# FuxiComputerVision/Nefii

Hardware: AMD Instinct MI355X
Metric: training rays/sec (Step-2 material opt) (higher is better)
Workload: dtype f16x3; 1 GPU; cfg3; parallelism=dp1, trace_tier=True, bracket_staged_eval=False, split_fp8=False, step_graph=False, cycle_batches=4, trace_prefetch=3, nonfinite_steps=0

## Files before the change

### include/nefii_amd.h

```cpp
#ifndef NEFII_AMD_H
#define NEFII_AMD_H

#include <stddef.h>
#include <stdint.h>

#ifdef __cplusplus
extern "C" {
#endif

#define NEFII_ABI_VERSION 18
#define NEFII_MAX_LAYERS 12
#define NEFII_TILE_ROWS 32
#define NEFII_MAX_WIDTH 512
#define NEFII_MAX_ENC 96
#define NEFII_MAX_LOBES 512

enum { NEFII_ACT_RELU = 0, NEFII_ACT_ELU = 1, NEFII_ACT_SOFTPLUS100 = 2 };
enum { NEFII_HEAD_NONE = 0, NEFII_HEAD_TANH01 = 1, NEFII_HEAD_POW2 = 2, NEFII_HEAD_SIGMOID = 3,
       NEFII_HEAD_RELU = 4, NEFII_HEAD_ABS = 5, NEFII_HEAD_RELU_INIT = 6 };
enum { NEFII_E_ARG = -1, NEFII_E_SHAPE = -2, NEFII_E_UNSUPPORTED = -3 };

typedef struct nefii_layer {
    int32_t k_x, k_e;
    int32_t n_out;
    int32_t n_pad;
    const float *w_fwd;
    const float *w_bwd;
    const float *bias;
    const void *w_f16x3;
    const void *w_bwd_f16x3;
} nefii_layer;

typedef struct nefii_mlp {
    int32_t n_layers;
    int32_t act;
    int32_t head;
    int32_t enc_freqs[3];
    int32_t feat_width;
    int32_t reserved;
    const void *w_stream;
    nefii_layer layer[NEFII_MAX_LAYERS];
} nefii_mlp;

int nefii_abi_version(void);

int nefii_padded_width(int v);

int nefii_pack_linear(const float *W, const float *bias, int n_out, int k_in,
                      int x_src0, int x_len, int e_src0, int e_len, float scale,
                      float *w_fwd, float *w_bwd, float *bias_pad, void *stream);

int nefii_pack_linear_f16x3(const float *W, int n_out, int k_in, int x_src0, int x_len, int e_src0, int e_len,
                            float scale, void *w_f16x3, void *stream);

typedef struct nefii_pack_source {
    const float *W;
    const float *bias;
    int32_t n_out, k_in, x_src0, x_len, e_src0, e_len;
    float scale;
    int32_t skip_f32;
} nefii_pack_source;
int nefii_pack_mlp(const nefii_mlp *h_mlp, const nefii_pack_source *h_layers, void *stream);

int nefii_mlp_forward(const nefii_mlp *h_mlp, const float *in_a, const float *in_b, const float *in_c,
                      const float *feat, int64_t n, float *out, int out_stride,
                      float *hidden_out, int hid_stride, float *stash, int stash_stride, void *stream);

int nefii_mlp_backward(const nefii_mlp *h_mlp, const float *d_out, int out_stride, const float *stash,
                       int stash_stride, int64_t n, float *dz, int dz_stride, void *stream);

int nefii_mlp_wgrad(const float *dz, int dz_stride, const float *x, int x_stride, int64_t n, int n_out, int k_in,
                    float scale, float *dW, float *db, void *stream);

int nefii_mlp_forward_f16(const nefii_mlp *h_mlp, const float *in_a, const float *in_b, const float *in_c,
                          const float *feat, int64_t n, float *out, int out_stride,
                          float *hidden_out, int hid_stride, float *stash, int stash_stride, int single_pass,
                          void *stream);
int nefii_mlp_grad_scale(const float *d_out, int64_t count, float *scale, void *stream);
int nefii_mlp_grad_scale_head(const float *d_out, int out_stride, const float *pre, int pre_stride, int64_t n, int n_out,
                              int head, float *scale, void *stream);
int nefii_mlp_backward_f16(const nefii_mlp *h_mlp, const float *d_out, int out_stride, const float *stash,
                           int stash_stride, int64_t n, float *dz, int dz_stride, const float *scale, void *stream);
int nefii_mlp_wgrad_f16(const float *dz, int dz_stride, const float *x, int x_stride, int64_t n, int n_out, int k_in,
                        float scale, const float *gscale, float *dW, float *db, void *stream);

int nefii_mlp_h16_supported(const nefii_mlp *h_mlp);
int nefii_mlp_x0_width(const nefii_mlp *h_mlp);
int nefii_mlp_forward_f16h(const nefii_mlp *h_mlp, const float *in_a, const float *in_b, const float *in_c,
                           const float *feat, int64_t n, float *out, int out_stride, float *hidden_out, int hid_stride,
                           void *stash16, int stash_stride, float *z_last, void *x0_16, void *stream);
int nefii_mlp_backward_f16h(const nefii_mlp *h_mlp, const float *d_out, int out_stride, const void *stash16,
                            int stash_stride, const float *z_last, int64_t n, void *dz16, int dz_stride,
                            const float *scale, void *stream);
int nefii_mlp_wgrad_f16h(const void *dz16, int dz_stride, const void *x, int x_stride, int x_half, int64_t n, int n_out,
                         int k_in, float scale, const float *gscale, float *dW, float *db, void *stream);

#define NEFII_MAX_WGRAD_ITEMS 12
typedef struct nefii_wgrad_item {
    const void *dz16;
    const void *x;
    float *dW, *db;
    int32_t dz_stride, x_stride, x_half, n_out, k_in;
    float scale;
} nefii_wgrad_item;
int nefii_mlp_wgrad_f16h_batch(const nefii_wgrad_item *h_items, int n_items, int64_t n, const float *gscale, void *stream);

int nefii_encode_inputs(const nefii_mlp *h_mlp, const float *in_a, const float *in_b, const float *in_c,
                        const float *feat, int64_t n, float *out, int width, void *stream);

int nefii_sdf_value_grad(const nefii_mlp *h_mlp, const float *x, int64_t n, float *sdf_out, int out_stride,
                         float *feat_out, int feat_stride, float *grad_out, float *ws, void *stream);
size_t nefii_sdf_value_grad_workspace_bytes(const nefii_mlp *h_mlp, int64_t n);

typedef struct nefii_tracer_params {
    float object_bounding_sphere, sdf_threshold, line_search_step;
    int32_t line_step_iters, sphere_tracing_iters, n_steps, n_rootfind_steps;
    int32_t training;
    int32_t bisect_levels;
    int32_t precision;
    float coarse_tau;
    int32_t coarse_cap;
    int32_t minsdf_group;
    int32_t small_round;
    int32_t trace_tier;
    float tier_kappa;
    float tier_gate;
    float minsdf_lipschitz;
    int32_t unread_misses;
    int32_t split_fp8;
} nefii_tracer_params;
#define NEFII_TRACE_COUNTERS 14
#define NEFII_CNT_SINGLES 0
#define NEFII_CNT_DENSE_ROWS 1
#define NEFII_CNT_BISECT_RAYS 2
#define NEFII_CNT_BISECT_USED 3
#define NEFII_CNT_REFINED 4
#define NEFII_CNT_COARSE_WINDOWS 5
#define NEFII_CNT_SEARCHES 6
#define NEFII_CNT_BISECT_EVALS 7
#define NEFII_CNT_TAU_AUDIT 8
#define NEFII_CNT_COARSE_SINGLES 9
#define NEFII_CNT_REPEATS 10
#define NEFII_CNT_COARSE_SAMPLES 11
#define NEFII_CNT_LIP_AUDIT 12
#define NEFII_CNT_PROBES 13

size_t nefii_sdf_stream_bytes(const nefii_mlp *h_sdf);
int nefii_pack_sdf_stream(const nefii_mlp *h_sdf, void *w_stream, void *stream);

size_t nefii_mlp_stream_bytes(const nefii_mlp *h_mlp);
int nefii_pack_mlp_stream(const nefii_mlp *h_mlp, void *w_stream, void *stream);

int nefii_pack_linear_f16x3_bwd(const float *W, int n_out, int k_in, int x_src0, int x_len, int e_src0, int e_len,
                                float scale, void *w_bwd_f16x3, void *stream);

int nefii_sdf_eval(const nefii_mlp *h_sdf, const float *x, int64_t n, float *sdf_out, void *stream);
int nefii_sdf_eval_coarse(const nefii_mlp *h_sdf, const float *x, int64_t n, float *sdf_out, void *stream);
int nefii_sdf_coarse_supported(const nefii_mlp *h_sdf);
int nefii_sdf_eval_fp8corr(const nefii_mlp *h_sdf, const float *x, int64_t n, float *sdf_out, void *stream);
int nefii_sdf_fp8corr_supported(const nefii_mlp *h_sdf);

size_t nefii_trace_workspace_bytes(int64_t n_rays, const nefii_tracer_params *h_params);
int nefii_trace_max_rounds(const nefii_tracer_params *h_params);
int nefii_trace_rays(const nefii_mlp *h_sdf, const nefii_tracer_params *h_params,
                     const float *origins, const float *dirs, const uint8_t *object_mask, int64_t n_rays,
                     const float *lin_steps, const float *minsdf_steps,
                     float *out_points, uint8_t *out_hit, float *out_dists,
                     void *workspace, size_t workspace_bytes, int32_t *counters, void *stream);

int nefii_trace_rays_rounds(const nefii_mlp *h_sdf, const nefii_tracer_params *h_params,
                            const float *origins, const float *dirs, const uint8_t *object_mask, int64_t n_rays,
                            const float *lin_steps, const float *minsdf_steps,
                            float *out_points, uint8_t *out_hit, float *out_dists,
                            void *workspace, size_t workspace_bytes, int32_t *counters,
                            int round_begin, int round_end, void *stream);
int nefii_trace_rays_groups(const nefii_mlp *h_sdf, const nefii_tracer_params *h_params,
                            const float *origins, const float *dirs, const uint8_t *object_mask,
                            int n_groups, const int64_t *group_begin,
                            const float *lin_steps, const float *minsdf_steps,
                            float *out_points, uint8_t *out_hit, float *out_dists,
                            void *const *workspaces, const size_t *workspace_bytes, int32_t *counters,
                            int round_begin, int round_end, void *const *streams);

#define NEFII_BOUND_GRID_MAX 640
size_t nefii_sdf_bound_grid_workspace_bytes(int G);
int nefii_sdf_bound_grid_build(const nefii_mlp *h_sdf, int G, float radius, float tau, float L_floor, float safety,
                               void *out_cells, void *workspace, void *stream);
int nefii_trace_rays_rounds_grid(const nefii_mlp *h_sdf, const nefii_tracer_params *h_params,
                                 const float *origins, const float *dirs, const uint8_t *object_mask, int64_t n_rays,
                                 const float *lin_steps, const float *minsdf_steps,
                                 float *out_points, uint8_t *out_hit, float *out_dists,
                                 void *workspace, size_t workspace_bytes, int32_t *counters,
                                 int round_begin, int round_end, const void *cells, int G, void *stream);
int nefii_trace_rays_groups_grid(const nefii_mlp *h_sdf, const nefii_tracer_params *h_params,
                                 const float *origins, const float *dirs, const uint8_t *object_mask,
                                 int n_groups, const int64_t *group_begin,
                                 const float *lin_steps, const float *minsdf_steps,
                                 float *out_points, uint8_t *out_hit, float *out_dists,
                                 void *const *workspaces, const size_t *workspace_bytes, int32_t *counters,
                                 int round_begin, int round_end, const void *cells, int G, void *const *streams);

int nefii_trace_profile_enable(int on);
int nefii_trace_profile_read(double *h_eval_ms, int *h_n_eval, double *h_span_ms);
int nefii_trace_profile_launches(float *h_ms, int cap);

int nefii_camera_rays(const float *uv, const float *pose, const float *intrinsics, int batch, int64_t samples,
                      float *out_dirs, float *out_origins, void *stream);


int nefii_sg_render_forward(const float *lgtSGs, int n_lobes, const float *specular, const float *roughness,
                            const float *albedo, const float *normal, const float *view, int64_t n,
                            float *rgb, float *spec_rgb, float *diff_rgb, void *stream);
int nefii_sg_render_backward(const float *lgtSGs, int n_lobes, const float *specular, const float *roughness,
                             const float *albedo, const float *normal, const float *view, int64_t n,
                             const float *d_rgb, const float *d_spec, const float *d_diff,
                             float *g_albedo, float *g_roughness, float *g_specular, float *g_lgtSGs, void *stream);

int nefii_env_radiance_forward(const float *lgtSGs, int n_lobes, const float *dirs, int64_t n, float eps,
                               float *rgb, void *stream);
int nefii_env_radiance_backward(const float *lgtSGs, int n_lobes, const float *dirs, int64_t n, float eps,
                                const float *d_rgb, float *g_lgtSGs, void *stream);

int64_t nefii_envfit_workspace_bytes(int64_t n, int n_lobes);
int nefii_envfit_loss_grad(const float *lgtSGs, int n_lobes, const float *dirs, const float *target, int64_t n, float eps,
                           void *workspace, float *loss, float *g_lgtSGs, float *rgb, void *stream);
int nefii_envfit_adam(float *lgtSGs, float *exp_avg, float *exp_avg_sq, int n_lobes, const float *dirs,
                      const float *target, int64_t n, float eps, double lr, double beta1, double beta2,
                      double adam_eps, int64_t step0, int iters, void *workspace, float *losses, void *stream);

int64_t nefii_mcubes_workspace_bytes(int nx, int ny, int nz);
int nefii_mcubes_count(const float *vol, int nx, int ny, int nz, float level, void *workspace, int64_t *counts,
                       void *stream);
int nefii_mcubes_emit(const float *vol, int nx, int ny, int nz, float level, float origin_x, float origin_y,
                      float origin_z, float spacing_x, float spacing_y, float spacing_z, void *workspace, float *verts,
                      int64_t max_verts, int *faces, int64_t max_tris, void *stream);

int nefii_mis_sample(const float *lgtSGs, int n_lobes, const float *roughness, const float *normal, const float *view,
                     const float *uniforms, int64_t n, float *wi, float *own_pdf, float *pdf_table, void *stream);

int64_t nefii_envlight_table_bytes(int height, int width);
int nefii_envlight_build(const float *map, int height, int width, void *table, void *stream);
int nefii_envlight_mis_sample(const float *map, const void *table, int height, int width, int coord,
                              const float *roughness, const float *normal, const float *view, const float *uniforms,
                              int64_t n, float *wi, float *own_pdf, float *pdf_table, float *light, void *stream);
int nefii_envlight_radiance(const float *map, int height, int width, int coord, const float *dirs, int64_t n,
                            float *rgb, void *stream);
int nefii_envlight_pdf(const void *table, int height, int width, int coord, const float *dirs, int64_t n, float *pdf,
                       void *stream);

int nefii_envlight_bounce_sample(const float *map, const void *table, int height, int width, int coord,
                                 const float *specular, const float *roughness, const float *albedo,
                                 const float *normal, const float *view, const float *uniforms, int64_t m, float *wo,
                                 float *weight, float *mix_pdf, void *stream);

int nefii_envlight_mis_sample_rot(const float *map, const void *table, int height, int width, int coord,
                                  const float *rot, const int *rot_identity, int A, const float *roughness,
                                  const float *normal, const float *view, const float *uniforms, int64_t n, float *wi,
                                  float *own_pdf, float *pdf_table, float *light, void *stream);
int nefii_envlight_bounce_sample_rot(const float *map, const void *table, int height, int width, int coord,
                                     const float *rot, const int *rot_identity, int A, const int *rot_index,
                                     const float *specular, const float *roughness, const float *albedo,
                                     const float *normal, const float *view, const float *uniforms, int64_t m,
                                     float *wo, float *weight, float *mix_pdf, void *stream);
int nefii_envlight_radiance_rot(const float *map, int height, int width, int coord, const float *rot,
                                const int *rot_identity, int A, const int *rot_index, const float *dirs, int64_t n,
                                float *rgb, void *stream);
int nefii_envlight_pdf_rot(const void *table, int height, int width, int coord, const float *rot,
                           const int *rot_identity, int A, const int *rot_index, const float *dirs, int64_t n,
                           float *pdf, void *stream);

int nefii_denoise_atrous(const void *guides0, const void *guides1, const void *in, void *out, int n_signals, int height,
                         int width, int step, float sigma_n, float sigma_x, float sigma_c_level, void *stream);

int nefii_mesh_sdf_query(const double *node_box, int64_t n_leaves_pow2, const double *tris ,
                         int64_t n_tris, int leaf_size, const double *points, int64_t n_points, int want_sign, double *out,
                         void *stream);

int nefii_mesh_cc_init(int32_t *parent, int64_t n_verts, int32_t *flags, void *stream);
int nefii_mesh_cc_round(const int32_t *faces, int64_t n_faces, int32_t *parent, int64_t n_verts, int32_t *flags,
                        void *stream);

int nefii_mesh_cluster_quadrics(const float *verts, int64_t n_verts, const int32_t *faces, int64_t n_faces,
                                const int32_t *cluster, const int32_t *corners, const int64_t *seg, const double *centre,
                                int64_t n_clusters, double h, double eps, double clamp, float *pos, int32_t *flags,
                                void *stream);

int64_t nefii_image_metrics_workspace_bytes(int B, int H, int W, int C, int levels);
int nefii_image_metrics(const float *x, const float *y, int B, int H, int W, int C, int levels, const double *window,
                        double c1, double c2, void *workspace, double *stats, double *sq_err, void *stream);

int nefii_mc_shade_forward(const float *specular, const float *roughness, const float *albedo, const float *normal,
                           const float *view, const float *wi, const float *own_pdf, const float *pdf_table,
                           const float *light, const float *visibility, const float *indirect, int64_t n,
                           float *rgb, float *spec_rgb, float *diff_rgb, void *stream);
int nefii_mc_shade_backward(const float *specular, const float *roughness, const float *albedo, const float *normal,
                            const float *view, const float *wi, const float *own_pdf, const float *pdf_table,
                            const float *light, const float *visibility, const float *indirect, int64_t n,
                            const float *d_rgb, const float *d_spec, const float *d_diff, float *g_light,
                            float *g_indirect, float *g_albedo, float *g_roughness, float *g_specular, void *stream);

typedef struct nefii_loss_params {
    float idr_rgb_weight, sg_rgb_weight, mask_weight, alpha, normalsmooth_weight, background_rgb_weight;
    int32_t loss_type;
    int32_t env_loss_type;
    int32_t r_patch;
    int32_t reserved;
} nefii_loss_params;
int nefii_idr_loss(const nefii_loss_params *h_params, const float *idr_rgb, const float *sg_rgb, const float *rgb_gt,
                   const uint8_t *network_object_mask, const uint8_t *object_mask, const float *sdf_output,
                   const float *normals, int64_t n, float *losses, float *d_idr_rgb, float *d_sg_rgb, void *stream);

#define NEFII_PATCH_WINDOW 11
typedef struct nefii_patch_loss_params {
    float idr_ssim_weight, sg_ssim_weight, roughnesssmooth_weight;
    int32_t r_patch;
    float window[NEFII_PATCH_WINDOW];
    int32_t reserved;
} nefii_patch_loss_params;
int64_t nefii_idr_patch_loss_workspace_bytes(const nefii_patch_loss_params *h_params, int64_t n);
int nefii_idr_patch_loss(const nefii_patch_loss_params *h_params, const float *idr_rgb, const float *sg_rgb,
                         const float *rgb_gt, const uint8_t *network_object_mask, const uint8_t *object_mask,
                         const float *roughness, const float *normals, int64_t n, void *workspace, float *losses,
                         float *d_idr_rgb, float *d_sg_rgb, float *d_roughness, void *stream);

#define NEFII_MAX_ROW_BLOCKS 12
typedef struct nefii_row_block {
    const float *src;
    float *dst;
    int32_t cols;
    int32_t src_row_stride;
    float fill;
    int32_t reserved;
} nefii_row_block;
int nefii_assemble_rows(const nefii_row_block *h_blocks, int n_blocks, const int64_t *where, int64_t n_src, int64_t rows,
                        void *stream);
int nefii_gather_rows(const nefii_row_block *h_blocks, int n_blocks, const int64_t *where, int64_t n_src, int64_t rows,
                      void *stream);

int nefii_prepare_hits(const float *points, const float *ray_dirs, const float *grad, const float *feat_src, int feat_cols,
                       const int64_t *where, int64_t n, int64_t rows, float *pts_out, float *view_out, float *nrm_out,
                       float *feat_out, void *stream);

int nefii_material_head_global(const float *rough_param, const float *spec_param, int n_spec, int fake_rough, int fake_spec,
                               float *rough_out, float *spec_out, void *stream);
int nefii_material_head_global_backward(const float *rough_param, const float *spec_param, int n_spec, int fake_rough,
                                        int fake_spec, const float *d_rough, const float *d_spec, float *g_rough_param,
                                        float *g_spec_param, void *stream);

int nefii_mfma_sustained_probe(int groups, float *h_ms, double *h_flops, void *stream);
int nefii_mfma_sustained_probe_chains(int groups, int chains, float *h_ms, double *h_flops, void *stream);

#ifdef __cplusplus
}
#endif
#endif
```

### nefii_amd/_lib.py

```python
import ctypes
import os

HERE = os.path.dirname(os.path.abspath(__file__))
LIB_PATH = os.environ.get('NEFII_LIB_PATH', os.path.join(HERE, 'csrc', 'libnefii_hip.so'))

MAX_LAYERS = 12
TILE_ROWS = 32
MAX_WIDTH = 512
MAX_ENC = 96
ABI_VERSION = 18
TRACE_COUNTERS = 14
(CNT_SINGLES, CNT_DENSE_ROWS, CNT_BISECT_RAYS, CNT_BISECT_USED, CNT_REFINED, CNT_COARSE_WINDOWS, CNT_SEARCHES, CNT_BISECT_EVALS,
 CNT_TAU_AUDIT, CNT_COARSE_SINGLES, CNT_REPEATS, CNT_COARSE_SAMPLES, CNT_LIP_AUDIT, CNT_PROBES) = range(TRACE_COUNTERS)
CNT_WORK = [CNT_SINGLES, CNT_DENSE_ROWS, CNT_BISECT_RAYS, CNT_REFINED, CNT_COARSE_WINDOWS, CNT_COARSE_SINGLES, CNT_COARSE_SAMPLES]
CNT_MAXIMA = [CNT_TAU_AUDIT, CNT_LIP_AUDIT]
TRACE_WS_FLOAT_ARRAYS = 13
TRACE_ITER_SHIFT = 20

ACT_RELU, ACT_ELU, ACT_SOFTPLUS100 = 0, 1, 2
HEAD_NONE, HEAD_TANH01, HEAD_POW2, HEAD_SIGMOID, HEAD_RELU, HEAD_ABS, HEAD_RELU_INIT = range(7)

c_float_p = ctypes.c_void_p


class Layer(ctypes.Structure):
    _fields_ = [('k_x', ctypes.c_int32), ('k_e', ctypes.c_int32), ('n_out', ctypes.c_int32),
                ('n_pad', ctypes.c_int32), ('w_fwd', ctypes.c_void_p), ('w_bwd', ctypes.c_void_p),
                ('bias', ctypes.c_void_p), ('w_f16x3', ctypes.c_void_p), ('w_bwd_f16x3', ctypes.c_void_p)]


class Mlp(ctypes.Structure):
    _fields_ = [('n_layers', ctypes.c_int32), ('act', ctypes.c_int32), ('head', ctypes.c_int32),
                ('enc_freqs', ctypes.c_int32 * 3), ('feat_width', ctypes.c_int32), ('reserved', ctypes.c_int32),
                ('w_stream', ctypes.c_void_p), ('layer', Layer * MAX_LAYERS)]


class TracerParams(ctypes.Structure):
    _fields_ = [('object_bounding_sphere', ctypes.c_float), ('sdf_threshold', ctypes.c_float),
                ('line_search_step', ctypes.c_float), ('line_step_iters', ctypes.c_int32),
                ('sphere_tracing_iters', ctypes.c_int32), ('n_steps', ctypes.c_int32),
                ('n_rootfind_steps', ctypes.c_int32), ('training', ctypes.c_int32), ('bisect_levels', ctypes.c_int32),
                ('precision', ctypes.c_int32), ('coarse_tau', ctypes.c_float), ('coarse_cap', ctypes.c_int32),
                ('minsdf_group', ctypes.c_int32), ('small_round', ctypes.c_int32), ('trace_tier', ctypes.c_int32),
                ('tier_kappa', ctypes.c_float), ('tier_gate', ctypes.c_float), ('minsdf_lipschitz', ctypes.c_float),
                ('unread_misses', ctypes.c_int32), ('split_fp8', ctypes.c_int32)]


class PackSource(ctypes.Structure):
    _fields_ = [('W', ctypes.c_void_p), ('bias', ctypes.c_void_p), ('n_out', ctypes.c_int32), ('k_in', ctypes.c_int32),
                ('x_src0', ctypes.c_int32), ('x_len', ctypes.c_int32), ('e_src0', ctypes.c_int32), ('e_len', ctypes.c_int32),
                ('scale', ctypes.c_float), ('skip_f32', ctypes.c_int32)]


class WgradItem(ctypes.Structure):
    _fields_ = [('dz16', ctypes.c_void_p), ('x', ctypes.c_void_p), ('dW', ctypes.c_void_p), ('db', ctypes.c_void_p),
                ('dz_stride', ctypes.c_int32), ('x_stride', ctypes.c_int32), ('x_half', ctypes.c_int32),
                ('n_out', ctypes.c_int32), ('k_in', ctypes.c_int32), ('scale', ctypes.c_float)]


MAX_WGRAD_ITEMS = 12


class RowBlock(ctypes.Structure):
    _fields_ = [('src', ctypes.c_void_p), ('dst', ctypes.c_void_p), ('cols', ctypes.c_int32), ('src_row_stride', ctypes.c_int32),
                ('fill', ctypes.c_float), ('reserved', ctypes.c_int32)]


MAX_ROW_BLOCKS = 12


class LossParams(ctypes.Structure):
    _fields_ = [('idr_rgb_weight', ctypes.c_float), ('sg_rgb_weight', ctypes.c_float), ('mask_weight', ctypes.c_float),
                ('alpha', ctypes.c_float), ('normalsmooth_weight', ctypes.c_float),
                ('background_rgb_weight', ctypes.c_float), ('loss_type', ctypes.c_int32),
                ('env_loss_type', ctypes.c_int32), ('r_patch', ctypes.c_int32), ('reserved', ctypes.c_int32)]


PATCH_WINDOW = 11


class PatchLossParams(ctypes.Structure):
    _fields_ = [('idr_ssim_weight', ctypes.c_float), ('sg_ssim_weight', ctypes.c_float),
                ('roughnesssmooth_weight', ctypes.c_float), ('r_patch', ctypes.c_int32),
                ('window', ctypes.c_float * PATCH_WINDOW), ('reserved', ctypes.c_int32)]


P = ctypes.c_void_p
I = ctypes.c_int
I64 = ctypes.c_int64
F = ctypes.c_float
D = ctypes.c_double

SIGNATURES = {
    'nefii_abi_version': (I, []),
    'nefii_padded_width': (I, [I]),
    'nefii_pack_linear': (I, [P, P, I, I, I, I, I, I, F, P, P, P, P]),
    'nefii_pack_linear_f16x3': (I, [P, I, I, I, I, I, I, F, P, P]),
    'nefii_pack_linear_f16x3_bwd': (I, [P, I, I, I, I, I, I, F, P, P]),
    'nefii_pack_mlp': (I, [ctypes.POINTER(Mlp), ctypes.POINTER(PackSource), P]),
    'nefii_mlp_forward': (I, [ctypes.POINTER(Mlp), P, P, P, P, I64, P, I, P, I, P, I, P]),
    'nefii_mlp_backward': (I, [ctypes.POINTER(Mlp), P, I, P, I, I64, P, I, P]),
    'nefii_mlp_wgrad': (I, [P, I, P, I, I64, I, I, F, P, P, P]),
    'nefii_mlp_forward_f16': (I, [ctypes.POINTER(Mlp), P, P, P, P, I64, P, I, P, I, P, I, I, P]),
    'nefii_mlp_grad_scale': (I, [P, I64, P, P]),
    'nefii_mlp_grad_scale_head': (I, [P, I, P, I, I64, I, I, P, P]),
    'nefii_mlp_backward_f16': (I, [ctypes.POINTER(Mlp), P, I, P, I, I64, P, I, P, P]),
    'nefii_mlp_wgrad_f16': (I, [P, I, P, I, I64, I, I, F, P, P, P, P]),
    'nefii_mlp_h16_supported': (I, [ctypes.POINTER(Mlp)]),
    'nefii_mlp_x0_width': (I, [ctypes.POINTER(Mlp)]),
    'nefii_mlp_forward_f16h': (I, [ctypes.POINTER(Mlp), P, P, P, P, I64, P, I, P, I, P, I, P, P, P]),
    'nefii_mlp_backward_f16h': (I, [ctypes.POINTER(Mlp), P, I, P, I, P, I64, P, I, P, P]),
    'nefii_mlp_wgrad_f16h': (I, [P, I, P, I, I, I64, I, I, F, P, P, P, P]),
    'nefii_mlp_wgrad_f16h_batch': (I, [ctypes.POINTER(WgradItem), I, I64, P, P]),
    'nefii_encode_inputs': (I, [ctypes.POINTER(Mlp), P, P, P, P, I64, P, I, P]),
    'nefii_sdf_value_grad': (I, [ctypes.POINTER(Mlp), P, I64, P, I, P, I, P, P, P]),
    'nefii_sdf_value_grad_workspace_bytes': (ctypes.c_size_t, [ctypes.POINTER(Mlp), I64]),
    'nefii_sdf_stream_bytes': (ctypes.c_size_t, [ctypes.POINTER(Mlp)]),
    'nefii_pack_sdf_stream': (I, [ctypes.POINTER(Mlp), P, P]),
    'nefii_mlp_stream_bytes': (ctypes.c_size_t, [ctypes.POINTER(Mlp)]),
    'nefii_pack_mlp_stream': (I, [ctypes.POINTER(Mlp), P, P]),
    'nefii_sdf_eval': (I, [ctypes.POINTER(Mlp), P, I64, P, P]),
    'nefii_sdf_eval_coarse': (I, [ctypes.POINTER(Mlp), P, I64, P, P]),
    'nefii_sdf_coarse_supported': (I, [ctypes.POINTER(Mlp)]),
    'nefii_sdf_eval_fp8corr': (I, [ctypes.POINTER(Mlp), P, I64, P, P]),
    'nefii_sdf_fp8corr_supported': (I, [ctypes.POINTER(Mlp)]),
    'nefii_trace_workspace_bytes': (ctypes.c_size_t, [I64, ctypes.POINTER(TracerParams)]),
    'nefii_trace_max_rounds': (I, [ctypes.POINTER(TracerParams)]),
    'nefii_trace_rays': (I, [ctypes.POINTER(Mlp), ctypes.POINTER(TracerParams), P, P, P, I64, P, P, P, P, P, P,
                             ctypes.c_size_t, P, P]),
    'nefii_trace_rays_rounds': (I, [ctypes.POINTER(Mlp), ctypes.POINTER(TracerParams), P, P, P, I64, P, P, P, P, P, P,
                                    ctypes.c_size_t, P, I, I, P]),
    'nefii_trace_rays_groups': (I, [ctypes.POINTER(Mlp), ctypes.POINTER(TracerParams), P, P, P, I, P, P, P, P, P, P, P, P,
                                    P, I, I, P]),
    'nefii_sdf_bound_grid_workspace_bytes': (ctypes.c_size_t, [I]),
    'nefii_sdf_bound_grid_build': (I, [ctypes.POINTER(Mlp), I, F, F, F, F, P, P, P]),
    'nefii_trace_rays_rounds_grid': (I, [ctypes.POINTER(Mlp), ctypes.POINTER(TracerParams), P, P, P, I64, P, P, P, P, P, P,
                                         ctypes.c_size_t, P, I, I, P, I, P]),
    'nefii_trace_rays_groups_grid': (I, [ctypes.POINTER(Mlp), ctypes.POINTER(TracerParams), P, P, P, I, P, P, P, P, P, P, P, P,
                                         P, I, I, P, I, P]),
    'nefii_trace_profile_enable': (I, [I]),
    'nefii_trace_profile_read': (I, [ctypes.POINTER(ctypes.c_double), ctypes.POINTER(I), ctypes.POINTER(ctypes.c_double)]),
    'nefii_trace_profile_launches': (I, [ctypes.POINTER(ctypes.c_float), I]),
    'nefii_idr_loss': (I, [ctypes.POINTER(LossParams), P, P, P, P, P, P, P, I64, P, P, P, P]),
    'nefii_idr_patch_loss_workspace_bytes': (I64, [ctypes.POINTER(PatchLossParams), I64]),
    'nefii_idr_patch_loss': (I, [ctypes.POINTER(PatchLossParams), P, P, P, P, P, P, P, I64, P, P, P, P, P, P]),
    'nefii_camera_rays': (I, [P, P, P, I, I64, P, P, P]),
    'nefii_assemble_rows': (I, [ctypes.POINTER(RowBlock), I, P, I64, I64, P]),
    'nefii_gather_rows': (I, [ctypes.POINTER(RowBlock), I, P, I64, I64, P]),
    'nefii_prepare_hits': (I, [P, P, P, P, I, P, I64, I64, P, P, P, P, P]),
    'nefii_material_head_global': (I, [P, P, I, I, I, P, P, P]),
    'nefii_material_head_global_backward': (I, [P, P, I, I, I, P, P, P, P, P]),
    'nefii_sg_render_forward': (I, [P, I, P, P, P, P, P, I64, P, P, P, P]),
    'nefii_sg_render_backward': (I, [P, I, P, P, P, P, P, I64, P, P, P, P, P, P, P, P]),
    'nefii_env_radiance_forward': (I, [P, I, P, I64, F, P, P]),
    'nefii_env_radiance_backward': (I, [P, I, P, I64, F, P, P, P]),
    'nefii_envfit_workspace_bytes': (I64, [I64, I]),
    'nefii_envfit_loss_grad': (I, [P, I, P, P, I64, F, P, P, P, P, P]),
    'nefii_envfit_adam': (I, [P, P, P, I, P, P, I64, F, D, D, D, D, I64, I, P, P, P]),
    'nefii_mcubes_workspace_bytes': (I64, [I, I, I]),
    'nefii_mcubes_count': (I, [P, I, I, I, F, P, P, P]),
    'nefii_mcubes_emit': (I, [P, I, I, I, F, F, F, F, F, F, F, P, P, I64, P, I64, P]),
    'nefii_mis_sample': (I, [P, I, P, P, P, P, I64, P, P, P, P]),
    'nefii_envlight_table_bytes': (I64, [I, I]),
    'nefii_envlight_build': (I, [P, I, I, P, P]),
    'nefii_envlight_mis_sample': (I, [P, P, I, I, I, P, P, P, P, I64, P, P, P, P, P]),
    'nefii_envlight_bounce_sample': (I, [P, P, I, I, I, P, P, P, P, P, P, I64, P, P, P, P]),
    'nefii_envlight_radiance': (I, [P, I, I, I, P, I64, P, P]),
    'nefii_envlight_pdf': (I, [P, I, I, I, P, I64, P, P]),
    'nefii_envlight_mis_sample_rot': (I, [P, P, I, I, I, P, P, I, P, P, P, P, I64, P, P, P, P, P]),
    'nefii_envlight_bounce_sample_rot': (I, [P, P, I, I, I, P, P, I, P, P, P, P, P, P, P, I64, P, P, P, P]),
    'nefii_envlight_radiance_rot': (I, [P, I, I, I, P, P, I, P, P, I64, P, P]),
    'nefii_envlight_pdf_rot': (I, [P, I, I, I, P, P, I, P, P, I64, P, P]),
    'nefii_denoise_atrous': (I, [P, P, P, P, I, I, I, I, F, F, F, P]),
    'nefii_image_metrics_workspace_bytes': (I64, [I, I, I, I, I]),
    'nefii_image_metrics': (I, [P, P, I, I, I, I, I, ctypes.POINTER(D), D, D, P, P, P, P]),
    'nefii_mesh_sdf_query': (I, [P, I64, P, I64, I, P, I64, I, P, P]),
    'nefii_mesh_cc_init': (I, [P, I64, P, P]),
    'nefii_mesh_cc_round': (I, [P, I64, P, I64, P, P]),
    'nefii_mesh_cluster_quadrics': (I, [P, I64, P, I64, P, P, P, P, I64, D, D, D, P, P, P]),
    'nefii_mc_shade_forward': (I, [P] * 11 + [I64, P, P, P, P]),
    'nefii_mc_shade_backward': (I, [P] * 11 + [I64] + [P] * 9),
    'nefii_mfma_sustained_probe': (I, [I, ctypes.POINTER(ctypes.c_float), ctypes.POINTER(ctypes.c_double), P]),
    'nefii_mfma_sustained_probe_chains': (I, [I, I, ctypes.POINTER(ctypes.c_float), ctypes.POINTER(ctypes.c_double), P]),
}

_lib = None


class NefiiLibraryError(RuntimeError):
    pass


def lib():
    global _lib
    if _lib is not None:
        return _lib
    if not os.path.exists(LIB_PATH):
        raise NefiiLibraryError(
            'libnefii_hip.so is not built (%s missing). Run `python -m nefii_amd.build`. '
            'There is no CPU/PyTorch fallback for the hot path.' % LIB_PATH)
    import torch
    try:
        handle = ctypes.CDLL(LIB_PATH)
    except OSError as e:
        raise NefiiLibraryError('cannot load %s: %s' % (LIB_PATH, e))
    for name, (res, args) in SIGNATURES.items():
        try:
            fn = getattr(handle, name)
        except AttributeError:
            raise NefiiLibraryError('%s does not export %s' % (LIB_PATH, name))
        fn.restype = res
        fn.argtypes = args
    if handle.nefii_abi_version() != ABI_VERSION:
        raise NefiiLibraryError('ABI version mismatch')
    _lib = handle
    return _lib


def check(rc, what):
    if rc != 0:
        raise RuntimeError('%s failed with status %d (%s)' % (
            what, rc, {-1: 'bad argument', -2: 'bad shape', -3: 'unsupported'}.get(rc, 'hipError_t')))
```

### nefii_amd/csrc/nefii_tracer.hip

```cpp
#include <cstdlib>
#include <vector>

#include "mlp_tile.h"
#include "hip_check.h"

using namespace nefii;

namespace {

enum Phase : int { PH_DONE = 0, PH_TRACE = 1, PH_SAMPLER = 2, PH_BISECT = 3, PH_MINSDF = 4, PH_SAMPLER_C = 5, PH_MINSDF_C = 6,
                   PH_SAMPLER_X = 7 };
constexpr int PH_POST = 100, PH_WAIT = -1;
constexpr int NCNT = NEFII_TRACE_COUNTERS;
constexpr int NEAR_PROBES = 6;
enum Kind : int { Q_START = 0, Q_END = 1, Q_MID = 2 };

constexpr int TRACE_WS_FLOAT_ARRAYS = 13, TRACE_ITER_SHIFT = 20;
struct RayState {
    float *t_s, *t_e, *cur_s, *cur_e, *nxt_s, *nxt_e, *t_min, *t_max, *res_s, *res_e, *lo, *hi, *mid;
    int *flags;
    float *big;
    unsigned *singles;
    unsigned *dense;
    unsigned *tri;
    unsigned *cdense;
    unsigned *refine;
    unsigned *csingles;
    int *block_live;
    unsigned *crefine;
    unsigned char *ord;
};
constexpr int CREF_CAP = 76;

constexpr int F_PHASE = 0x7;
constexpr int F_LIVE_S = 1 << 3, F_LIVE_E = 1 << 4, F_PEND_S = 1 << 5, F_PEND_E = 1 << 6;
constexpr int F_STEPPED = 1 << 7;
constexpr int F_SPH = 1 << 8, F_SAMP = 1 << 9, F_HIT = 1 << 10;
constexpr int F_OWN = 1 << 11;
constexpr int F_IT_SHIFT = 12, F_IT_MASK = 0xFF;
constexpr int F_K_SHIFT = TRACE_ITER_SHIFT, F_K_MASK = 0xF;
constexpr int F_WIN_SHIFT = 24, F_WIN_MASK = 0x7;
enum SamplerWin : int {
    SW_WHOLE_ROW = 0,
    SW_WINDOW_1 = 1, SW_WINDOW_2 = 2, SW_WINDOW_3 = 3, SW_WINDOW_4 = 4,
    SW_STAGE1 = 5, SW_STAGE2 = 6,
    SW_GRID = 7
};
enum MinSdfWin : int {
    MW_ROW_IN = 0,
    MW_SECOND = 1,
    MW_STAGE1 = 2, MW_STAGE2 = 3,
    MW_ENTER = 4,
    MW_SHARED = 5
};
__device__ __forceinline__ int win_of(int fl) { return (fl >> F_WIN_SHIFT) & F_WIN_MASK; }
__device__ __forceinline__ int with_win(int fl, int w) { return (fl & ~(F_WIN_MASK << F_WIN_SHIFT)) | (w << F_WIN_SHIFT); }
constexpr int CWIN_STAGE1 = 4;
constexpr int F_CRS_S = 1 << 27, F_CRS_E = 1 << 28, F_AUD_S = 1 << 29, F_AUD_E = 1 << 30;
__host__ __device__ __forceinline__ int coarse_window(int n_steps) { return (n_steps + 3) >> 2; }

__device__ __forceinline__ float fmul(float a, float b) { return __fmul_rn(a, b); }
__device__ __forceinline__ float fadd(float a, float b) { return __fadd_rn(a, b); }
__device__ __forceinline__ float fsub(float a, float b) { return __fsub_rn(a, b); }

struct Params {
    nefii_tracer_params p;
    int64_t n;
    const float *o, *d;
    const uint8_t *obj;
    const float *lin, *steps;
    float *out_pts, *out_dist;
    uint8_t *out_hit;
    int *counters;
    int levels, tri_nodes;
    float tau;
    int cap;
    int chunk;
    float chunk_gate;
    int window;
    float tier_band;
    float tier_gate;
    float lip;
    int share;
    int stage_bracket;
    int miss_argmin;
    const unsigned *cells;
    int grid_n;
    float grid_inv_h;
    RayState s;
};

__host__ __device__ __forceinline__ int stage1_count(int ns) { return coarse_window(ns); }
__host__ __device__ __forceinline__ int stage1_pos(int ns, int j) { return (j * (ns - 1)) / (stage1_count(ns) - 1); }
__device__ __forceinline__ bool staged_bracket(const Params &P, int64_t r) {
    return P.lip > 0.f && P.stage_bracket && (!P.p.training || P.obj[r] == 0);
}
__device__ __forceinline__ int minsdf_row(const Params &P, int64_t r) {
    const int g = P.p.minsdf_group;
    return g > 0 ? (int)(r / g) : 0;
}

__device__ __forceinline__ float minsdf_step(const Params &P, int64_t r, int i) {
    const int g = P.p.minsdf_group;
    return P.steps[(g > 0 ? (r / g) * (int64_t)P.p.n_steps : 0) + i];
}

struct Emit {
    bool qs, qe;
    bool cs, ce;
    bool qt, qd;
    int nc, cwin;
    unsigned dense_which;
    int consumed;
    int n_alg;
    int n_ref;
    unsigned cmask[4];
    int n_rep;
    bool ref_coarse;
    __device__ __forceinline__ void mark(int i) {
#pragma unroll
        for (int w = 0; w < 4; ++w) cmask[w] |= (i >> 5) == w ? 1u << (i & 31) : 0u;
    }
    __device__ __forceinline__ bool marked(int i) const {
        unsigned word = 0u;
#pragma unroll
        for (int w = 0; w < 4; ++w) word = (i >> 5) == w ? cmask[w] : word;
        return (word >> (i & 31)) & 1u;
    }
    __device__ __forceinline__ void clear_marks() { cmask[0] = cmask[1] = cmask[2] = cmask[3] = 0u; }
};
enum Total : int { T_SINGLES, T_DENSE, T_TRI, T_CONSUMED, T_REFINE, T_CWINDOWS, T_ALG, T_CSINGLES, T_REP, T_CREFINE, N_TOTALS };
enum List : int { L_SINGLES, L_DENSE, L_TRI, L_REFINE, L_CDENSE, L_CSINGLES, L_CREFINE, N_LISTS };

__device__ __forceinline__ void append_queries(const Params &P, int round, unsigned ray, const Emit &e) {
    __shared__ int wtot[N_TOTALS][4];
    __shared__ int base[N_LISTS];
    const bool qs = e.qs && !e.cs, qe = e.qe && !e.ce, qcs = e.qs && e.cs, qce = e.qe && e.ce;
    const int nc = e.nc, n_ref = e.n_ref;
    const bool ref_coarse = e.ref_coarse;
    const int lane = threadIdx.x & 63, wave = threadIdx.x >> 6;
    const unsigned long long bs = __ballot(qs), be = __ballot(qe), bt = __ballot(e.qt), bd = __ballot(e.qd);
    const unsigned long long bcs = __ballot(qcs), bce = __ballot(qce);
    const unsigned long long lt = (1ull << lane) - 1ull;
    int cons = e.consumed, alg = e.n_alg, rep = e.n_rep;
#pragma unroll
    for (int o = 32; o > 0; o >>= 1) cons += __shfl_xor(cons, o), alg += __shfl_xor(alg, o), rep += __shfl_xor(rep, o);
    int incl = ref_coarse ? 0 : n_ref;
    int incl2 = ref_coarse ? n_ref : 0;
#pragma unroll
    for (int o = 1; o < 64; o <<= 1) {
        const int t = __shfl_up(incl, o), t2 = __shfl_up(incl2, o);
        if (lane >= o) incl += t, incl2 += t2;
    }
    const int wref = __shfl(incl, 63), wref2 = __shfl(incl2, 63);
    int cincl = nc;
#pragma unroll
    for (int o = 1; o < 64; o <<= 1) {
        const int t = __shfl_up(cincl, o);
        if (lane >= o) cincl += t;
    }
    const int wcoarse = __shfl(cincl, 63);
    if (lane == 0) {
        wtot[T_SINGLES][wave] = __popcll(bs) + __popcll(be);
        wtot[T_DENSE][wave] = __popcll(bd);
        wtot[T_TRI][wave] = __popcll(bt);
        wtot[T_CONSUMED][wave] = cons;
        wtot[T_REFINE][wave] = wref;
        wtot[T_CWINDOWS][wave] = wcoarse;
        wtot[T_ALG][wave] = alg;
        wtot[T_CSINGLES][wave] = __popcll(bcs) + __popcll(bce);
        wtot[T_REP][wave] = rep;
        wtot[T_CREFINE][wave] = wref2;
    }
    __syncthreads();
    if (threadIdx.x == 0) {
        int t[N_TOTALS];
        for (int i = 0; i < N_TOTALS; ++i) t[i] = wtot[i][0] + wtot[i][1] + wtot[i][2] + wtot[i][3];
        int *cnt = P.counters + round * NCNT;
        base[L_SINGLES] = t[T_SINGLES] ? atomicAdd(&cnt[NEFII_CNT_SINGLES], t[T_SINGLES]) : 0;
        base[L_DENSE] = t[T_DENSE] ? atomicAdd(&cnt[NEFII_CNT_DENSE_ROWS], t[T_DENSE]) : 0;
        base[L_TRI] = t[T_TRI] ? atomicAdd(&cnt[NEFII_CNT_BISECT_RAYS], t[T_TRI]) : 0;
        if (t[T_CONSUMED]) atomicAdd(&cnt[NEFII_CNT_BISECT_USED], t[T_CONSUMED]);
        base[L_REFINE] = t[T_REFINE] ? atomicAdd(&cnt[NEFII_CNT_REFINED], t[T_REFINE]) : 0;
        base[L_CDENSE] = t[T_CWINDOWS] ? atomicAdd(&cnt[NEFII_CNT_COARSE_WINDOWS], t[T_CWINDOWS]) : 0;
        if (t[T_ALG]) atomicAdd(&cnt[NEFII_CNT_SEARCHES], t[T_ALG]);
        if (t[T_TRI]) atomicAdd(&cnt[NEFII_CNT_BISECT_EVALS], t[T_TRI] * P.tri_nodes);
        base[L_CSINGLES] = t[T_CSINGLES] ? atomicAdd(&cnt[NEFII_CNT_COARSE_SINGLES], t[T_CSINGLES]) : 0;
        if (t[T_REP]) atomicAdd(&cnt[NEFII_CNT_REPEATS], t[T_REP]);
        base[L_CREFINE] = t[T_CREFINE] ? atomicAdd(&cnt[NEFII_CNT_COARSE_SAMPLES], t[T_CREFINE]) : 0;
    }
    __syncthreads();
    int off_s = base[L_SINGLES], off_d = base[L_DENSE], off_t = base[L_TRI], off_r = base[L_REFINE], off_c = base[L_CDENSE],
        off_cs = base[L_CSINGLES], off_r2 = base[L_CREFINE];
    for (int w = 0; w < wave; ++w) {
        off_r2 += wtot[T_CREFINE][w];
        off_s += wtot[T_SINGLES][w];
        off_d += wtot[T_DENSE][w];
        off_t += wtot[T_TRI][w];
        off_r += wtot[T_REFINE][w];
        off_c += wtot[T_CWINDOWS][w];
        off_cs += wtot[T_CSINGLES][w];
    }
    if (qs) P.s.singles[off_s + __popcll(bs & lt)] = (ray << 2) | Q_START;
    if (qe) P.s.singles[off_s + __popcll(bs) + __popcll(be & lt)] = (ray << 2) | Q_END;
    if (qcs) P.s.csingles[off_cs + __popcll(bcs & lt)] = (ray << 2) | Q_START;
    if (qce) P.s.csingles[off_cs + __popcll(bcs) + __popcll(bce & lt)] = (ray << 2) | Q_END;
    if (e.qd) P.s.dense[off_d + __popcll(bd & lt)] = (ray << 1) | e.dense_which;
    if (e.qt) P.s.tri[off_t + __popcll(bt & lt)] = ray;
    for (int k = 0; k < nc; ++k)
        P.s.cdense[off_c + cincl - nc + k] = ((unsigned)(e.cwin + k) << 29) | (ray << 1) | e.dense_which;
    if (n_ref > 0) {
        size_t o = ref_coarse ? (size_t)off_r2 + incl2 - n_ref : (size_t)off_r + incl - n_ref;
        unsigned *list = ref_coarse ? P.s.crefine : P.s.refine;
#pragma unroll
        for (int w = 0; w < 4; ++w) {
            unsigned mbits = e.cmask[w];
            while (mbits) {
                const int bit = __ffs(mbits) - 1;
                mbits &= mbits - 1;
                list[o++] = (ray << 7) | (unsigned)(32 * w + bit);
            }
        }
    }
    __syncthreads();
}

__device__ __forceinline__ float tri_depth(float lo, float hi, int j) {
    const unsigned k = (unsigned)j + 1u;
    const int level = 31 - __clz(k);
    float mid = fmul(fadd(lo, hi), 0.5f);
    for (int b = level - 1; b >= 0; --b) {
        if ((k >> b) & 1u) lo = mid; else hi = mid;
        mid = fmul(fadd(lo, hi), 0.5f);
    }
    return mid;
}

__device__ __forceinline__ void finish(const Params &P, int64_t r, float dist, bool hit) {
    const float ox = P.o[r * 3], oy = P.o[r * 3 + 1], oz = P.o[r * 3 + 2];
    const float dx = P.d[r * 3], dy = P.d[r * 3 + 1], dz = P.d[r * 3 + 2];
    P.out_dist[r] = dist;
    P.out_hit[r] = hit ? 1 : 0;
    P.out_pts[r * 3] = fadd(ox, fmul(dist, dx));
    P.out_pts[r * 3 + 1] = fadd(oy, fmul(dist, dy));
    P.out_pts[r * 3 + 2] = fadd(oz, fmul(dist, dz));
}

__global__ __launch_bounds__(128) void minsdf_order_kernel(Params P) {
    const int ns = P.p.n_steps, i = threadIdx.x;
    if (i >= ns) return;
    const float *st = P.steps + (size_t)blockIdx.x * ns;
    const float si = st[i];
    int rank = 0;
    for (int j = 0; j < ns; ++j) {
        const float sj = st[j];
        rank += (sj < si || (sj == si && j < i)) ? 1 : 0;
    }
    P.s.ord[(size_t)blockIdx.x * ns + rank] = (unsigned char)i;
}


__device__ __forceinline__ int init_ray(const Params &P, int64_t r, int round, int &fl, Emit &e) {
    const bool tier = P.tier_band > 0.f;
    const float ox = P.o[r * 3], oy = P.o[r * 3 + 1], oz = P.o[r * 3 + 2];
    const float dx = P.d[r * 3], dy = P.d[r * 3 + 1], dz = P.d[r * 3 + 2];
    const float b = fadd(fadd(fmul(dx, ox), fmul(dy, oy)), fmul(dz, oz));
    const float nrm = sqrtf(fadd(fadd(fmul(ox, ox), fmul(oy, oy)), fmul(oz, oz)));
    const float rad = P.p.object_bounding_sphere;
    const float under = fsub(fmul(b, b), fsub(fmul(nrm, nrm), fmul(rad, rad)));
    const bool sph = under > 0.f;
    float t0 = 0.f, t1 = 0.f;
    if (sph) {
        const float sq = sqrtf(under);
        t0 = fmaxf(fsub(-sq, b), 0.01f);
        t1 = fmaxf(fsub(sq, b), 0.01f);
    }
    P.s.t_s[r] = t0;
    P.s.t_e[r] = t1;
    P.s.t_min[r] = t0;
    P.s.t_max[r] = t1;
    P.s.nxt_s[r] = 0.f;
    P.s.nxt_e[r] = 0.f;
    P.s.cur_s[r] = 0.f;
    P.s.cur_e[r] = 0.f;
    fl = PH_TRACE;
    if (!sph) return PH_TRACE;
    fl |= F_SPH | F_LIVE_S | F_LIVE_E | F_PEND_S | F_PEND_E;
    e.qs = e.qe = true;
    e.cs = tier && t0 > 0.01f;
    e.ce = tier && t1 > 0.01f;
    fl |= (e.cs ? F_CRS_S : 0) | (e.ce ? F_CRS_E : 0);
    P.s.flags[r] = fl;
    return PH_WAIT;
}

__device__ __forceinline__ void begin_stage1(const Params &P, int64_t r, int from, int stage_code, int &fl, Emit &e) {
    float *v = P.s.big + (size_t)r * P.p.n_steps;
    for (int i = from; i < P.p.n_steps; ++i) v[i] = __builtin_inff();
    e.nc = 1;
    e.cwin = CWIN_STAGE1;
    fl = with_win(fl, stage_code);
}

__device__ __forceinline__ bool grid_bounds(const Params &P, int64_t r, float t, float &lo, float &hi) {
    const float rad = P.p.object_bounding_sphere, g = (float)P.grid_n;
    const float ox = P.o[r * 3], oy = P.o[r * 3 + 1], oz = P.o[r * 3 + 2];
    const float dx = P.d[r * 3], dy = P.d[r * 3 + 1], dz = P.d[r * 3 + 2];
    const float fx = fmul(fadd(fadd(ox, fmul(t, dx)), rad), P.grid_inv_h);
    const float fy = fmul(fadd(fadd(oy, fmul(t, dy)), rad), P.grid_inv_h);
    const float fz = fmul(fadd(fadd(oz, fmul(t, dz)), rad), P.grid_inv_h);
    lo = -__builtin_inff(), hi = __builtin_inff();
    if (!(fx >= 0.f && fx < g && fy >= 0.f && fy < g && fz >= 0.f && fz < g)) return false;
    const unsigned w = P.cells[((size_t)(int)fx * P.grid_n + (size_t)(int)fy) * P.grid_n + (size_t)(int)fz];
    lo = (float)__builtin_bit_cast(_Float16, (unsigned short)(w & 0xFFFFu));
    hi = (float)__builtin_bit_cast(_Float16, (unsigned short)(w >> 16));
    return true;
}

__device__ __forceinline__ void begin_grid_bracket(const Params &P, int64_t r, int round, int from, int &fl, Emit &e) {
    const int ns = P.p.n_steps;
    float *v = P.s.big + (size_t)r * ns;
    const float a = P.s.t_s[r], rng = fsub(P.s.t_e[r], a);
    const bool obj = P.obj[r] != 0;
    int j1 = ns;
    float U = __builtin_inff(), lo0 = 0.f;
    for (int i = 0; i < ns; ++i) {
        float lo, hi;
        if (i < from)
            lo = hi = v[i];
        else
            grid_bounds(P, r, fadd(a, fmul(P.lin[i], rng)), lo, hi);
        if (hi < -P.tau && j1 == ns) j1 = i;
        U = fminf(U, hi);
        if (i == 0) lo0 = lo;
        if (i >= from) v[i] = lo;
    }
    const bool front_only = obj && j1 < ns && lo0 > 0.f;
    const bool sign_only = front_only || !P.miss_argmin;
    const float lim = sign_only ? 0.f : fmaxf(0.f, fadd(U, P.tau));
    const int last = front_only ? j1 : ns - 1;
    int k = 0, n_near = 0, probe = -1;
    unsigned probe_h = ~0u;
    for (int i = from; i < ns; ++i) {
        const float lb = v[i];
        v[i] = __builtin_inff();
        if (i > last) continue;
        if (!(fsub(lb, 1e-6f) > lim)) {
            e.mark(i);
            ++k;
        } else if (n_near < NEAR_PROBES && !(fsub(lb, 1e-6f) > fadd(lim, fmul(2.f, P.tau)))) {
            e.mark(i);
            ++k, ++n_near;
        } else {
            const unsigned h = ((unsigned)r * 2654435761u) ^ ((unsigned)(i + 1) * 0x9E3779B1u);
            const unsigned hh = (h ^ (h >> 15)) * 0x85EBCA6Bu;
            if (hh < probe_h) probe_h = hh, probe = i;
        }
    }
    if (probe >= 0) {
        e.mark(probe);
        ++k, ++n_near;
    }
    if (n_near > 0) atomicAdd(P.counters + round * NCNT + NEFII_CNT_PROBES, n_near);
    if (k > 0 && k <= CREF_CAP) {
        e.n_ref = k;
        e.ref_coarse = true;
        fl = with_win(fl, SW_GRID);
    } else {
        e.clear_marks();
        e.nc = 4;
    }
}

__device__ __forceinline__ void grid_audit(const Params &P, int64_t r, int round) {
    const int ns = P.p.n_steps;
    const float *v = P.s.big + (size_t)r * ns;
    const float a = P.s.t_s[r], rng = fsub(P.s.t_e[r], a);
    float worst = 0.f;
    for (int i = 0; i < ns; ++i) {
        if (!(v[i] < __builtin_inff())) continue;
        float lo, hi;
        if (!grid_bounds(P, r, fadd(a, fmul(P.lin[i], rng)), lo, hi)) continue;
        worst = fmaxf(worst, fmaxf(fsub(fsub(lo, P.tau), v[i]), fsub(v[i], fadd(hi, P.tau))));
    }
    if (worst > 0.f) atomicMax(P.counters + round * NCNT + NEFII_CNT_LIP_AUDIT, __float_as_int(worst));
}

__device__ __forceinline__ void begin_coarse_bracket(const Params &P, int64_t r, int round, int from, bool in_mask, int &fl, Emit &e) {
    if (staged_bracket(P, r) && P.cells && !P.p.training) {
        begin_grid_bracket(P, r, round, from, fl, e);
    } else if (staged_bracket(P, r)) {
        begin_stage1(P, r, from, SW_STAGE1, fl, e);
    } else if ((P.window & 1) && in_mask) {
        e.nc = 1;
        fl = with_win(fl, SW_WINDOW_1);
    } else {
        e.nc = 4;
    }
}

__device__ __forceinline__ int end_trace(const Params &P, int64_t r, int round, int &fl, Emit &e, float t_s, float t_e,
                                         float cur_s, float cur_e, bool live_s, int it) {
    const bool coarse = P.tau > 0.f;
    const bool hit = t_s < t_e;
    fl = (fl & F_SPH) | (hit ? F_HIT : 0) | (live_s ? F_SAMP : 0) | ((it & F_K_MASK) << F_K_SHIFT);
    P.s.t_s[r] = t_s;
    P.s.t_e[r] = t_e;
    if (!live_s) {
        P.s.mid[r] = t_s;
        return PH_POST;
    }
    const bool go_coarse = coarse && 0.5f * (cur_s + cur_e + (t_e - t_s)) > 3.f * P.tau;
    if (go_coarse && P.chunk > 0 && P.obj[r] != 0 &&
        cur_s <= P.chunk_gate * (float)(P.chunk - 1) * (t_e - t_s) / (float)(P.p.n_steps - 1)) {
        fl |= PH_SAMPLER_X;
        e.n_ref = P.chunk;
        e.cmask[0] = (1u << P.chunk) - 1u;
    } else {
        fl |= go_coarse ? PH_SAMPLER_C : PH_SAMPLER;
        e.qd = !go_coarse;
        if (go_coarse) begin_coarse_bracket(P, r, round, 0, P.obj[r] != 0, fl, e);
    }
    e.n_alg = 1;
    e.dense_which = 0;
    P.s.flags[r] = fl;
    return PH_WAIT;
}

__device__ __forceinline__ int step_trace(const Params &P, int64_t r, int round, int &fl, Emit &e) {
    const nefii_tracer_params &tp = P.p;
    const bool tier = P.tier_band > 0.f;
    const float thr = tp.sdf_threshold;
    float t_s = P.s.t_s[r], t_e = P.s.t_e[r];
    float cur_s = P.s.cur_s[r], cur_e = P.s.cur_e[r];
    float nxt_s = P.s.nxt_s[r], nxt_e = P.s.nxt_e[r];
    bool live_s = fl & F_LIVE_S, live_e = fl & F_LIVE_E;
    int it = (fl >> F_IT_SHIFT) & F_IT_MASK, k = (fl >> F_K_SHIFT) & F_K_MASK;
    if (fl & F_PEND_S) nxt_s = P.s.res_s[r];
    if (fl & F_PEND_E) nxt_e = P.s.res_e[r];
    fl &= ~(F_AUD_S | F_AUD_E);
    const bool rep_s = (fl & F_PEND_S) && (fl & F_CRS_S) && !(fabsf(nxt_s) > P.tier_band);
    const bool rep_e = (fl & F_PEND_E) && (fl & F_CRS_E) && !(fabsf(nxt_e) > P.tier_band);
    if (rep_s || rep_e) {
        if (rep_s) e.qs = true, fl = (fl & ~F_CRS_S) | F_AUD_S, ++e.n_rep;
        if (rep_e) e.qe = true, fl = (fl & ~F_CRS_E) | F_AUD_E, ++e.n_rep;
        P.s.flags[r] = fl;
        return PH_WAIT;
    }
    bool wait = false;
    fl &= ~(F_CRS_S | F_CRS_E);
    if (fl & F_STEPPED) {
        const bool bad_s = nxt_s < 0.f, bad_e = nxt_e < 0.f;
        if ((bad_s || bad_e) && k < tp.line_step_iters) {
            const float back = (1.f - tp.line_search_step) / (float)(1 << k);
            fl &= ~(F_PEND_S | F_PEND_E);
            if (bad_s) {
                t_s = fsub(t_s, fmul(back, cur_s));
                e.qs = true;
                e.cs = tier && back * cur_s > P.tier_gate;
                fl |= F_PEND_S | (e.cs ? F_CRS_S : 0);
            }
            if (bad_e) {
                t_e = fadd(t_e, fmul(back, cur_e));
                e.qe = true;
                e.ce = tier && back * cur_e > P.tier_gate;
                fl |= F_PEND_E | (e.ce ? F_CRS_E : 0);
            }
            ++k;
            wait = true;
        } else {
            live_s = live_s && (t_s < t_e);
            live_e = live_e && (t_s < t_e);
        }
    }
    if (!wait) {
        cur_s = live_s ? nxt_s : 0.f;
        if (cur_s <= thr) cur_s = 0.f;
        cur_e = live_e ? nxt_e : 0.f;
        if (cur_e <= thr) cur_e = 0.f;
        live_s = live_s && (cur_s > thr);
        live_e = live_e && (cur_e > thr);
        if (it == tp.sphere_tracing_iters || !(live_s || live_e)) return end_trace(P, r, round, fl, e, t_s, t_e, cur_s, cur_e, live_s, it);
        ++it;
        t_s = fadd(t_s, cur_s);
        t_e = fsub(t_e, cur_e);
        nxt_s = 0.f;
        nxt_e = 0.f;
        k = 0;
        fl &= ~(F_PEND_S | F_PEND_E);
        if (live_s) {
            e.qs = true;
            e.cs = tier && cur_s > P.tier_gate;
            fl |= F_PEND_S | (e.cs ? F_CRS_S : 0);
        }
        if (live_e) {
            e.qe = true;
            e.ce = tier && cur_e > P.tier_gate;
            fl |= F_PEND_E | (e.ce ? F_CRS_E : 0);
        }
        fl |= F_STEPPED;
    }
    fl &= ~(F_LIVE_S | F_LIVE_E | (F_IT_MASK << F_IT_SHIFT) | (F_K_MASK << F_K_SHIFT));
    fl |= (live_s ? F_LIVE_S : 0) | (live_e ? F_LIVE_E : 0) | (it << F_IT_SHIFT) | (k << F_K_SHIFT);
    P.s.t_s[r] = t_s;
    P.s.t_e[r] = t_e;
    P.s.cur_s[r] = cur_s;
    P.s.cur_e[r] = cur_e;
    P.s.nxt_s[r] = nxt_s;
    P.s.nxt_e[r] = nxt_e;
    P.s.flags[r] = fl;
    return PH_WAIT;
}

__device__ __forceinline__ int sampler_leading(const Params &P, int64_t r, int round, int &fl, Emit &e) {
    const int ns = P.p.n_steps;
    float *v = P.s.big + (size_t)r * ns;
    int ind = -1;
    for (int i = 0; i < P.chunk; ++i)
        if (v[i] < 0.f && ind < 0) ind = i;
    if (ind >= 1) {
        for (int i = P.chunk; i < ns; ++i) v[i] = 3.0e38f;
        return PH_SAMPLER;
    }
    fl = (fl & ~F_PHASE) | PH_SAMPLER_C;
    begin_coarse_bracket(P, r, round, P.chunk, true, fl, e);
    e.dense_which = 0;
    P.s.flags[r] = fl;
    return PH_WAIT;
}

template <typename Search>
__device__ __forceinline__ bool staged_walk(const Params &P, int64_t r, int round, int &fl, Emit &e, const float *v, float Llen,
                                            bool stage1, const Search &S) {
    const int ns = P.p.n_steps;
    int *cnt = P.counters + round * NCNT;
    int ja = 0, k = 0, n_near = 0;
    float worst = 0.f;
    int probe = -1;
    unsigned probe_h = ~0u;
    for (int kk = 1; kk < ns - 1; ++kk) {
        if (kk == stage1_pos(ns, ja + 1)) {
            ++ja;
            continue;
        }
        const int ia = S.sample(stage1_pos(ns, ja)), ib = S.sample(stage1_pos(ns, ja + 1)), is = S.sample(kk);
        const float sa = S.depth(ia), sb = S.depth(ib), ss = S.depth(is);
        const float lb = fsub(fmaxf(fsub(v[ia], fmul(Llen, fsub(ss, sa))), fsub(v[ib], fmul(Llen, fsub(sb, ss)))), P.tau);
        if (stage1) {
            if (S.skip(kk, v)) continue;
            if (!(fsub(lb, 1e-6f) > S.lim)) {
                e.mark(is);
                ++k;
            } else if (n_near < NEAR_PROBES && !(fsub(lb, 1e-6f) > fadd(S.lim, fmul(2.f, P.tau)))) {
                e.mark(is);
                ++k, ++n_near;
            } else {
                const unsigned h = ((unsigned)r * 2654435761u) ^ ((unsigned)(kk + 1) * 0x9E3779B1u);
                const unsigned hh = (h ^ (h >> 15)) * 0x85EBCA6Bu;
                if (hh < probe_h) probe_h = hh, probe = is;
            }
        } else if (v[is] < __builtin_inff()) {
            worst = fmaxf(worst, fsub(fsub(lb, P.tau), v[is]));
        }
    }
    fl = with_win(fl, 0);
    if (stage1 && probe >= 0) {
        e.mark(probe);
        ++k, ++n_near;
    }
    if (stage1 && n_near > 0) atomicAdd(cnt + NEFII_CNT_PROBES, n_near);
    if (stage1 && k > 0) {
        if (k <= CREF_CAP) {
            e.n_ref = k;
            e.ref_coarse = true;
            fl = with_win(fl, Search::STAGE2);
        } else {
            e.clear_marks();
            e.nc = 4;
            e.dense_which = Search::WHICH;
        }
        P.s.flags[r] = fl;
        return true;
    }
    if (worst > 0.f) atomicMax(cnt + NEFII_CNT_LIP_AUDIT, __float_as_int(worst));
    e.clear_marks();
    return false;
}

struct BracketSearch {
    const float *lin;
    float lim;
    int last;
    static constexpr int STAGE2 = SW_STAGE2;
    static constexpr unsigned WHICH = 0;
    __device__ __forceinline__ int sample(int k) const { return k; }
    __device__ __forceinline__ float depth(int i) const { return lin[i]; }
    __device__ __forceinline__ bool skip(int k, const float *v) const { return k >= last || v[k] < __builtin_inff(); }
};

struct MinSdfSearch {
    const Params &P;
    int64_t r;
    const unsigned char *ord;
    float lim;
    static constexpr int STAGE2 = MW_STAGE2;
    static constexpr unsigned WHICH = 1;
    __device__ __forceinline__ int sample(int k) const { return ord[k]; }
    __device__ __forceinline__ float depth(int i) const { return minsdf_step(P, r, i); }
    __device__ __forceinline__ bool skip(int, const float *) const { return false; }
};

__device__ __forceinline__ int sampler_staged(const Params &P, int64_t r, int round, int &fl, Emit &e) {
    const int ns = P.p.n_steps, n1 = stage1_count(ns);
    const float *v = P.s.big + (size_t)r * ns;
    if (win_of(fl) == SW_GRID) {
        grid_audit(P, r, round);
        fl = with_win(fl, SW_WHOLE_ROW);
        return PH_SAMPLER_C;
    }
    const float Llen = fmul(P.lip, fsub(P.s.t_e[r], P.s.t_s[r]));
    const bool obj = P.obj[r] != 0;
    float best = __builtin_inff();
    int j1 = ns;
    for (int j = 0; j < n1; ++j) {
        const int i = stage1_pos(ns, j);
        best = fminf(best, v[i]);
        if (v[i] < -P.tau && j1 == ns) j1 = i;
    }
    const bool front_only = obj && j1 < ns && !(v[0] < P.tau);
    const bool sign_only = front_only || !P.miss_argmin;
    const BracketSearch S = {P.lin, sign_only ? 0.f : fmaxf(0.f, fadd(best, P.tau)), front_only ? j1 : ns - 1};
    return staged_walk(P, r, round, fl, e, v, Llen, win_of(fl) == SW_STAGE1, S) ? PH_WAIT : PH_SAMPLER_C;
}

__device__ __forceinline__ int sampler_windows(const Params &P, int64_t r, int round, int &fl, Emit &e) {
    const int ns = P.p.n_steps, cw = coarse_window(ns);
    const int wn = win_of(fl);
    const int have = wn * cw < ns ? wn * cw : ns;
    float *v = P.s.big + (size_t)r * ns;
    int i0 = -1, i1 = -1;
    for (int i = 0; i < have; ++i) {
        const float x = v[i];
        if (x < P.tau && i0 < 0) i0 = i;
        if (x < -P.tau && i1 < 0) i1 = i;
    }
    if (i1 >= 0 && i0 > 0) {
        for (int i = have; i < ns; ++i) v[i] = 3.0e38f;
        fl = with_win(fl, SW_WHOLE_ROW);
    } else if (have < ns) {
        const bool rest = i0 == 0;
        e.nc = rest ? 4 - wn : 1;
        e.cwin = wn;
        fl = with_win(fl, rest ? SW_WINDOW_4 : wn + 1);
        e.dense_which = 0;
        P.s.flags[r] = fl;
        return PH_WAIT;
    } else {
        fl = with_win(fl, SW_WHOLE_ROW);
    }
    return PH_SAMPLER_C;
}

__device__ __forceinline__ int sampler_coarse(const Params &P, int64_t r, int round, int &fl, Emit &e) {
    const int ns = P.p.n_steps;
    const float tau = P.tau;
    const float *v = P.s.big + (size_t)r * ns;
    int i0 = -1, i1 = -1;
    float vmin = v[0];
    for (int i = 0; i < ns; ++i) {
        const float x = v[i];
        if (x < tau && i0 < 0) i0 = i;
        if (x < -tau && i1 < 0) i1 = i;
        vmin = x < vmin ? x : vmin;
    }
    const bool obj = P.obj[r] != 0;
    const bool need_argmin = P.miss_argmin && !(obj && i1 >= 0);
    int n_sign = 0, n_min = 0;
    if (i0 >= 0) {
        const int end = i1 >= 0 ? i1 : ns;
        for (int i = i0; i < end; ++i)
            if (v[i] < tau) {
                e.mark(i);
                ++n_sign;
            }
        if (i0 == 0 && fabsf(v[ns - 1]) < tau && !e.marked(ns - 1)) {
// ... 1404 lines not shown

int64_t minsdf_rows(int64_t n, const nefii_tracer_params *p) {
    return p->minsdf_group > 0 ? (n + p->minsdf_group - 1) / p->minsdf_group : 1;
}

size_t carve(RayState &s, char *base, int64_t n, int ns, int cap, int64_t step_rows) {
    size_t off = 0;
    auto take = [&](size_t bytes) {
        char *p = base ? base + off : nullptr;
        off += align256(bytes);
        return p;
    };
    float **fl[] = {&s.t_s, &s.t_e, &s.cur_s, &s.cur_e, &s.nxt_s, &s.nxt_e, &s.t_min,
                    &s.t_max, &s.res_s, &s.res_e, &s.lo, &s.hi, &s.mid};
    static_assert(sizeof(fl) / sizeof(fl[0]) == TRACE_WS_FLOAT_ARRAYS, "ops.trace_iterations finds the flags behind these");
    for (auto f : fl) *f = (float *)take(sizeof(float) * n);
    s.flags = (int *)take(sizeof(int) * n);
    s.big = (float *)take(sizeof(float) * (size_t)n * ns);
    s.singles = (unsigned *)take(sizeof(unsigned) * 2 * n);
    s.dense = (unsigned *)take(sizeof(unsigned) * n);
    s.tri = (unsigned *)take(sizeof(unsigned) * n);
    s.cdense = (unsigned *)take(sizeof(unsigned) * 4 * n);
    s.refine = (unsigned *)take(sizeof(unsigned) * (size_t)n * (cap > 0 ? cap : 0));
    s.csingles = (unsigned *)take(sizeof(unsigned) * 2 * n);
    s.block_live = (int *)take(sizeof(int) * ((n + 255) / 256));
    s.crefine = (unsigned *)take(step_rows > 0 ? sizeof(unsigned) * (size_t)n * CREF_CAP : 0);
    s.ord = (unsigned char *)take(step_rows > 0 ? (size_t)step_rows * ns : 0);
    return off;
}

}

namespace {
struct Prof {
    bool on = false;
    std::vector<hipEvent_t> ev;
    size_t used = 0;
    hipEvent_t t0 = nullptr, t1 = nullptr;
    bool have_span = false;
} g_prof;
hipEvent_t prof_event() {
    if (g_prof.used == g_prof.ev.size()) {
        hipEvent_t e;
        (void)hipEventCreate(&e);
        g_prof.ev.push_back(e);
    }
    return g_prof.ev[g_prof.used++];
}
}

extern "C" int nefii_trace_profile_enable(int on) {
    g_prof.on = on != 0;
    g_prof.used = 0;
    g_prof.have_span = false;
    return 0;
}

extern "C" int nefii_trace_profile_read(double *eval_ms, int *n_eval, double *span_ms) {
    double tot = 0.0;
    for (size_t i = 0; i + 1 < g_prof.used; i += 2) {
        hipError_t e = hipEventSynchronize(g_prof.ev[i + 1]);
        if (e != hipSuccess) return (int)e;
        float ms = 0.f;
        e = hipEventElapsedTime(&ms, g_prof.ev[i], g_prof.ev[i + 1]);
        if (e != hipSuccess) return (int)e;
        tot += ms;
    }
    if (eval_ms) *eval_ms = tot;
    if (n_eval) *n_eval = (int)(g_prof.used / 2);
    if (span_ms) {
        *span_ms = 0.0;
        if (g_prof.have_span) {
            (void)hipEventSynchronize(g_prof.t1);
            float ms = 0.f;
            (void)hipEventElapsedTime(&ms, g_prof.t0, g_prof.t1);
            *span_ms = ms;
        }
    }
    g_prof.used = 0;
    return 0;
}

extern "C" int nefii_trace_profile_launches(float *h_ms, int cap) {
    int n = 0;
    for (size_t i = 0; i + 1 < g_prof.used && n < cap; i += 2, ++n) {
        hipError_t e = hipEventSynchronize(g_prof.ev[i + 1]);
        if (e != hipSuccess) return -(int)e;
        float ms = 0.f;
        (void)hipEventElapsedTime(&ms, g_prof.ev[i], g_prof.ev[i + 1]);
        h_ms[n] = ms;
    }
    return n;
}

static size_t stream_bytes_1to4(const nefii_mlp *h_sdf) {
    size_t units_vg = 0;
    if (vg_shape(h_sdf)) units_vg = (size_t)stream_steps(h_sdf) + vg_units_bwd(h_sdf);
    return (size_t)8 * (stream_steps(h_sdf) + stream_steps8(h_sdf) + units_vg) * 256 * sizeof(half8) +
           (size_t)8 * stream_steps_sp(h_sdf) * shape16p(h_sdf) * 64 * sizeof(half8);
}
int stream_steps_f8(const nefii_mlp *m) {
    if (shape16p(m) != 4 || m->reserved != 1) return 0;
    int G = 0;
    for (int l = 0; l < m->n_layers - 1; ++l) G += 8 * f_chunks(m->layer[l]);
    return G;
}

extern "C" size_t nefii_sdf_stream_bytes(const nefii_mlp *h_sdf) {
    if (!h_sdf || h_sdf->n_layers < 2 || h_sdf->n_layers > NEFII_MAX_LAYERS || !shape16p(h_sdf)) return 0;
    return stream_bytes_1to4(h_sdf) + (size_t)8 * stream_steps_f8(h_sdf) * 4096;
}

extern "C" int nefii_sdf_fp8corr_supported(const nefii_mlp *h_sdf) {
    return h_sdf && h_sdf->w_stream && h_sdf->n_layers >= 2 && h_sdf->n_layers <= NEFII_MAX_LAYERS && stream_steps_f8(h_sdf) > 0;
}

__global__ void pack_sdf_stream_f8_kernel(nefii_mlp m, half8 *__restrict__ dst, int G) {
    const int g = blockIdx.x, wave = blockIdx.y;
    int l = 0, u = g;
    while (u >= 8 * f_chunks(m.layer[l])) u -= 8 * f_chunks(m.layer[l]), ++l;
    const half8 *w = reinterpret_cast<const half8 *>(m.layer[l].w_f16x3);
    const int NT = m.layer[l].n_pad >> 5, K16 = (m.layer[l].k_x + m.layer[l].k_e) >> 4;
    const int c = u >> 3, j = u & 7;
    const int i = threadIdx.x >> 6, lane = threadIdx.x & 63, kg = lane >> 4;
    half8 v;
    for (int e = 0; e < 8; ++e) v[e] = (_Float16)0.f;
    if (j < 4) {
        const int s = 4 * c + j, n = 64 * wave + 16 * i + (lane & 15);
        const int s16 = 2 * s + (kg >> 1), t = n >> 5, lane_src = (n & 31) + 32 * (kg & 1);
        if (s16 < K16) v = w[(((size_t)s16 * NT + t) * 2) * 64 + lane_src];
    } else {
        const int ft = j - 4, part = i >> 1, n = 64 * wave + 16 * ft + (lane & 15), t = n >> 5;
        const int k0 = 128 * c + 32 * kg + 16 * (i & 1), s16 = k0 >> 4;
        const float sc = f8_scale(part == 0 ? F8_WL_E : F8_WH_E);
        int out[4] = {0, 0, 0, 0};
        if (s16 < K16) {
            const half8 a = w[(((size_t)s16 * NT + t) * 2 + (part == 0 ? 1 : 0)) * 64 + (n & 31)];
            const half8 b = w[(((size_t)s16 * NT + t) * 2 + (part == 0 ? 1 : 0)) * 64 + (n & 31) + 32];
            out[0] = f8_pack4((float)a[0] * sc, (float)a[1] * sc, (float)a[2] * sc, (float)a[3] * sc);
            out[1] = f8_pack4((float)a[4] * sc, (float)a[5] * sc, (float)a[6] * sc, (float)a[7] * sc);
            out[2] = f8_pack4((float)b[0] * sc, (float)b[1] * sc, (float)b[2] * sc, (float)b[3] * sc);
            out[3] = f8_pack4((float)b[4] * sc, (float)b[5] * sc, (float)b[6] * sc, (float)b[7] * sc);
        }
        const i32x4 o4 = {out[0], out[1], out[2], out[3]};
        v = __builtin_bit_cast(half8, o4);
    }
    dst[((size_t)wave * G + g) * 256 + threadIdx.x] = v;
}

extern "C" int nefii_sdf_coarse_supported(const nefii_mlp *h_sdf) {
    return h_sdf && h_sdf->w_stream && h_sdf->n_layers >= 2 && h_sdf->n_layers <= NEFII_MAX_LAYERS &&
           stream_steps_sp(h_sdf) > 0;
}

extern "C" int nefii_pack_sdf_stream(const nefii_mlp *h_sdf, void *w_stream, void *stream) {
    if (!h_sdf || !w_stream) return NEFII_E_ARG;
    if (nefii_sdf_stream_bytes(h_sdf) == 0) return NEFII_E_UNSUPPORTED;
    for (int l = 0; l < h_sdf->n_layers - 1; ++l)
        if (!h_sdf->layer[l].w_f16x3) return NEFII_E_ARG;
    const int G = stream_steps(h_sdf);
    hipLaunchKernelGGL(pack_sdf_stream_kernel, dim3(G, 8), dim3(256), 0, (hipStream_t)stream, *h_sdf, (half8 *)w_stream, G,
                       shape16p(h_sdf), 0);
    HIP_CHECK_LAUNCH();
    const int G8 = stream_steps8(h_sdf);
    if (G8 > 0) {
        hipLaunchKernelGGL(pack_sdf_stream_kernel, dim3(G8, 8), dim3(256), 0, (hipStream_t)stream, *h_sdf,
                           (half8 *)w_stream + (size_t)8 * G * 256, G8, 4, 1);
        HIP_CHECK_LAUNCH();
    }
    const int Gs = stream_steps_sp(h_sdf);
    if (Gs > 0) {
        const int ft = shape16p(h_sdf);
        hipLaunchKernelGGL(pack_sdf_stream_sp_kernel, dim3(Gs, 8), dim3(64 * ft), 0, (hipStream_t)stream, *h_sdf,
                           (half8 *)w_stream + (size_t)8 * (G + G8) * 256, Gs, ft);
        HIP_CHECK_LAUNCH();
    }
    if (const int ft = vg_shape(h_sdf)) {
        const int Gb = vg_units_bwd(h_sdf), Gw = G + Gb;
        half8 *dst = (half8 *)w_stream + vg_stream_offset(h_sdf);
        hipLaunchKernelGGL(pack_sdf_stream_kernel, dim3(G, 8), dim3(256), 0, (hipStream_t)stream, *h_sdf, dst, Gw, ft, 0);
        HIP_CHECK_LAUNCH();
        hipLaunchKernelGGL(pack_sdf_stream_bwd_kernel, dim3(Gb, 8), dim3(256), 0, (hipStream_t)stream, *h_sdf, dst, Gw, G, ft);
        HIP_CHECK_LAUNCH();
    }
    if (const int Gf = stream_steps_f8(h_sdf)) {
        hipLaunchKernelGGL(pack_sdf_stream_f8_kernel, dim3(Gf, 8), dim3(256), 0, (hipStream_t)stream, *h_sdf,
                           reinterpret_cast<half8 *>((char *)w_stream + stream_bytes_1to4(h_sdf)), Gf);
        HIP_CHECK_LAUNCH();
    }
    return 0;
}

namespace nefii {
static int vg_grid(int64_t n, int rows) {
    const int64_t n_tiles = (n + rows - 1) / rows;
    return (int)(n_tiles < 256 ? (n_tiles > 0 ? n_tiles : 1) : 256);
}
static bool vg_enabled() {
    static const bool v = env_int("NEFII_VG_STREAM", 1) != 0;
    return v;
}
size_t value_grad_stream_ws_bytes(const nefii_mlp *m, int64_t n) {
    if (!m || n <= 0 || !m->w_stream || !vg_enabled()) return 0;
    const int ft = vg_shape(m);
    if (!ft) return 0;
    const int rows = ft == 4 ? 64 : 96;
    return (size_t)vg_grid(n, rows) * (m->n_layers - 1) * 8 * (ft * rows / 16) * 64 * sizeof(float4v);
}
int value_grad_stream_launch(const nefii_mlp *m, const float *x, int64_t n, float *sdf_out, int out_stride, float *feat_out,
                             int feat_stride, float *grad_out, float *ws, hipStream_t st) {
    const int ft = m->w_stream && vg_enabled() ? vg_shape(m) : 0;
    if (!ft) return NEFII_E_UNSUPPORTED;
    const int Gw = stream_steps(m) + vg_units_bwd(m);
    if (ft == 4)
        hipLaunchKernelGGL((sdf_value_grad16q_kernel<4, 4>), dim3(vg_grid(n, 64)), dim3(512), 0, st, *m, x, n, sdf_out, out_stride,
                           feat_out, feat_stride, grad_out, reinterpret_cast<float4v *>(ws), vg_stream_offset(m), Gw);
    else
        hipLaunchKernelGGL((sdf_value_grad16q_kernel<6, 2>), dim3(vg_grid(n, 96)), dim3(512), 0, st, *m, x, n, sdf_out, out_stride,
                           feat_out, feat_stride, grad_out, reinterpret_cast<float4v *>(ws), vg_stream_offset(m), Gw);
    HIP_CHECK_LAUNCH();
    return 0;
}
}

static unsigned coarse_d_grid() {
    static const int g = env_int("NEFII_COARSE_D_GRID", 0);
    return (unsigned)(g > 0 ? g : 256);
}
static int coarse_two_groups() {
    static const int v = env_int("NEFII_COARSE_D", 0);
    return v;
}
static int coarse_qt() {
    static const int q = env_int("NEFII_COARSE_QT", 0);
    return q == 4 || q == 6 || q == 8 ? q : 0;
}
static int coarse_rows(int ft) {
    const int q = coarse_qt();
    if (ft == 2) return 96;
    return 16 * (q ? q : 4);
}
static dim3 points_grid(int64_t n, int rows) {
    const int64_t n_tiles = (n + rows - 1) / rows;
    return dim3((int)(n_tiles < 512 ? n_tiles : 512));
}
#define NEFII_COARSE_LAUNCH(KERNEL, KERNEL_D, ft, grid, st, ...)                                                    \
    do {                                                                                                            \
        const int rows_ = coarse_rows(ft);                                                                          \
        if ((ft) == 2)                                                                                              \
            hipLaunchKernelGGL((KERNEL<6, 2>), grid, dim3(512), 0, st, __VA_ARGS__);                                \
        else if (rows_ == 64 && coarse_two_groups())                                                                \
            hipLaunchKernelGGL((KERNEL_D<4>), dim3((grid).x < coarse_d_grid() ? (grid).x : coarse_d_grid()), dim3(512), 0, st, \
                               __VA_ARGS__);                                                                    \
        else if (rows_ == 64)                                                                                       \
            hipLaunchKernelGGL((KERNEL<4, 4>), grid, dim3(512), 0, st, __VA_ARGS__);                                \
        else if (rows_ == 96)                                                                                       \
            hipLaunchKernelGGL((KERNEL<6, 4, false>), grid, dim3(512), 0, st, __VA_ARGS__);                         \
        else                                                                                                        \
            hipLaunchKernelGGL((KERNEL<8, 4, false>), grid, dim3(512), 0, st, __VA_ARGS__);                         \
    } while (0)

extern "C" int nefii_sdf_eval_coarse(const nefii_mlp *h_sdf, const float *x, int64_t n, float *sdf_out, void *stream) {
    if (!h_sdf || h_sdf->n_layers < 1 || h_sdf->n_layers > NEFII_MAX_LAYERS) return NEFII_E_ARG;
    if (!nefii_sdf_coarse_supported(h_sdf)) return NEFII_E_UNSUPPORTED;
    if (n <= 0) return 0;
    if (!x || !sdf_out) return NEFII_E_ARG;
    if (!sdf_net_ok(h_sdf)) return NEFII_E_UNSUPPORTED;
    const int ft = shape16p(h_sdf);
    const dim3 grid = points_grid(n, coarse_rows(ft));
    NEFII_COARSE_LAUNCH(sdf_points_kernel16s, sdf_points_kernel16d, ft, grid, (hipStream_t)stream, *h_sdf, x, n, sdf_out);
    HIP_CHECK_LAUNCH();
    return 0;
}

namespace {
constexpr int GRID_SLAB = 8;

__global__ __launch_bounds__(256) void grid_points_kernel(int G, float radius, float h, int i0, int planes, float *__restrict__ x) {
    const int V = G + 1;
    const int64_t n = (int64_t)planes * V * V;
    for (int64_t q = (int64_t)blockIdx.x * blockDim.x + threadIdx.x; q < n; q += (int64_t)gridDim.x * blockDim.x) {
        const int k = (int)(q % V), j = (int)((q / V) % V), i = i0 + (int)(q / ((int64_t)V * V));
        x[q * 3] = fadd(-radius, fmul((float)i, h));
        x[q * 3 + 1] = fadd(-radius, fmul((float)j, h));
        x[q * 3 + 2] = fadd(-radius, fmul((float)k, h));
    }
}

__device__ __forceinline__ unsigned short half_toward(float x, bool up) {
    const _Float16 hv = (_Float16)x;
    unsigned short bits = __builtin_bit_cast(unsigned short, hv);
    const bool wrong = up ? (float)hv < x : (float)hv > x;
    if (wrong) {
        const bool pos = !(bits & 0x8000u);
        if ((bits & 0x7FFFu) == 0)
            bits = up ? 0x0001u : 0x8001u;
        else
            bits = (unsigned short)(pos == up ? bits + 1 : bits - 1);
    }
    return bits;
}

__global__ __launch_bounds__(256) void grid_cells_kernel(int G, float h, float tau, float l_floor, float safety,
                                                         const float *__restrict__ g, unsigned *__restrict__ cells) {
    const int V = G + 1;
    const int64_t n = (int64_t)G * G * G;
    const float reach = (float)((double)h * 0.8660254037844386);
    for (int64_t c = (int64_t)blockIdx.x * blockDim.x + threadIdx.x; c < n; c += (int64_t)gridDim.x * blockDim.x) {
        const int k = (int)(c % G), j = (int)((c / G) % G), i = (int)(c / ((int64_t)G * G));
        auto at = [&](int a, int b, int d) { return g[((int64_t)a * V + b) * V + d]; };
        float lo = __builtin_inff(), hi = -__builtin_inff(), slope = 0.f;
        for (int a = i - 1; a <= i + 2; ++a)
            for (int b = j - 1; b <= j + 2; ++b)
                for (int d = k - 1; d <= k + 2; ++d) {
                    if (a < 0 || a > G || b < 0 || b > G || d < 0 || d > G) continue;
                    const float v = at(a, b, d);
                    if (a >= i && a <= i + 1 && b >= j && b <= j + 1 && d >= k && d <= k + 1) lo = fminf(lo, v), hi = fmaxf(hi, v);
                    if (a < i + 2 && a < G) slope = fmaxf(slope, __fdiv_rn(fabsf(fsub(at(a + 1, b, d), v)), h));
                    if (b < j + 2 && b < G) slope = fmaxf(slope, __fdiv_rn(fabsf(fsub(at(a, b + 1, d), v)), h));
                    if (d < k + 2 && d < G) slope = fmaxf(slope, __fdiv_rn(fabsf(fsub(at(a, b, d + 1), v)), h));
                }
        const float lcell = fmaxf(fmul(safety, slope), l_floor);
        const float slack = fadd(tau, fmul(lcell, reach));
        cells[c] = (unsigned)half_toward(fsub(lo, slack), false) | ((unsigned)half_toward(fadd(hi, slack), true) << 16);
    }
}
}

extern "C" size_t nefii_sdf_bound_grid_workspace_bytes(int G) {
    if (G < 2 || G > NEFII_BOUND_GRID_MAX) return 0;
    const size_t V = (size_t)G + 1;
    return align256(sizeof(float) * V * V * V) + align256(sizeof(float) * 3 * GRID_SLAB * V * V);
}

extern "C" int nefii_sdf_bound_grid_build(const nefii_mlp *h_sdf, int G, float radius, float tau, float L_floor, float safety,
                                          void *out_cells, void *workspace, void *stream) {
    if (!h_sdf || !out_cells || !workspace || h_sdf->n_layers < 1 || h_sdf->n_layers > NEFII_MAX_LAYERS) return NEFII_E_ARG;
    if (!(radius > 0.f && radius < 1e6f) || !(tau >= 0.f && tau < 1e6f) || !(L_floor > 0.f && L_floor < 1e6f) ||
        !(safety > 0.f && safety < 1e6f))
        return NEFII_E_ARG;
    if (G < 2 || G > NEFII_BOUND_GRID_MAX) return NEFII_E_SHAPE;
    if (!nefii_sdf_coarse_supported(h_sdf) || !sdf_net_ok(h_sdf)) return NEFII_E_UNSUPPORTED;
    hipStream_t st = (hipStream_t)stream;
    const int V = G + 1;
    const float h = (float)(2.0 * (double)radius / (double)G);
    float *g = (float *)workspace;
    float *x = (float *)((char *)workspace + align256(sizeof(float) * (size_t)V * V * V));
    const int ft = shape16p(h_sdf);
    for (int i0 = 0; i0 < V; i0 += GRID_SLAB) {
        const int planes = V - i0 < GRID_SLAB ? V - i0 : GRID_SLAB;
        const int64_t n = (int64_t)planes * V * V;
        hipLaunchKernelGGL(grid_points_kernel, dim3((int)((n + 255) / 256 < 1024 ? (n + 255) / 256 : 1024)), dim3(256), 0, st, G,
                           radius, h, i0, planes, x);
        HIP_CHECK_LAUNCH();
        const dim3 grid = points_grid(n, coarse_rows(ft));
        float *out = g + (size_t)i0 * V * V;
        NEFII_COARSE_LAUNCH(sdf_points_kernel16s, sdf_points_kernel16d, ft, grid, st, *h_sdf, (const float *)x, n, out);
        HIP_CHECK_LAUNCH();
    }
    const int64_t n_cells = (int64_t)G * G * G;
    hipLaunchKernelGGL(grid_cells_kernel, dim3((int)((n_cells + 255) / 256 < 4096 ? (n_cells + 255) / 256 : 4096)), dim3(256), 0,
                       st, G, h, tau, L_floor, safety, (const float *)g, (unsigned *)out_cells);
    HIP_CHECK_LAUNCH();
    return 0;
}

extern "C" int nefii_sdf_eval_fp8corr(const nefii_mlp *h_sdf, const float *x, int64_t n, float *sdf_out, void *stream) {
    if (!h_sdf || !x || !sdf_out || n < 0) return NEFII_E_ARG;
    if (!nefii_sdf_fp8corr_supported(h_sdf)) return NEFII_E_UNSUPPORTED;
    for (int l = 0; l < h_sdf->n_layers; ++l)
        if (!h_sdf->layer[l].w_f16x3) return NEFII_E_ARG;
    if (n == 0) return 0;
    hipLaunchKernelGGL(sdf_points_kernel16f, points_grid(n, 64), dim3(512), 0, (hipStream_t)stream, *h_sdf, x, n, sdf_out,
                       (const void *)((const char *)h_sdf->w_stream + stream_bytes_1to4(h_sdf)));
    HIP_CHECK_LAUNCH();
    return 0;
}

extern "C" int nefii_sdf_eval(const nefii_mlp *h_sdf, const float *x, int64_t n, float *sdf_out, void *stream) {
    if (!h_sdf || h_sdf->n_layers < 1 || h_sdf->n_layers > NEFII_MAX_LAYERS) return NEFII_E_ARG;
    if (n <= 0) return 0;
    if (!x || !sdf_out) return NEFII_E_ARG;
    if (!sdf_net_ok(h_sdf)) return NEFII_E_UNSUPPORTED;
    for (int l = 0; l < h_sdf->n_layers; ++l)
        if (!h_sdf->layer[l].w_f16x3 || !h_sdf->layer[l].bias) return NEFII_E_ARG;
    const dim3 grid = points_grid(n, TILE_W);
    hipStream_t st = (hipStream_t)stream;
    const int ft = fits16p(h_sdf);
    if (ft == 2)
        hipLaunchKernelGGL(sdf_points_kernel16q<2>, grid, dim3(512), 0, st, *h_sdf, x, n, sdf_out);
    else if (ft && h_sdf->reserved == 1)
        hipLaunchKernelGGL(sdf_points_kernel16q<4>, grid, dim3(512), 0, st, *h_sdf, x, n, sdf_out);
    else if (ft)
        hipLaunchKernelGGL(sdf_points_kernel16p<P16W>, grid, dim3(64 * P16W), 0, st, *h_sdf, x, n, sdf_out);
    else
        hipLaunchKernelGGL(sdf_points_kernel16w, grid, dim3(WG_W), 0, st, *h_sdf, x, n, sdf_out);
    HIP_CHECK_LAUNCH();
    return 0;
}

static int coarse_cap(const nefii_tracer_params *p) {
    if (!(p->coarse_tau > 0.f)) return 0;
    const int c = p->coarse_cap <= 0 ? 64 : p->coarse_cap;
    return c > 100 ? 100 : c;
}

static bool minsdf_staged(const nefii_tracer_params *p) {
    return p->coarse_tau > 0.f && p->minsdf_lipschitz > 0.f && p->n_steps >= 16 && p->n_steps <= 128;
}

static int trace_rounds(const nefii_tracer_params *p) {
    const int trace = 1 + p->sphere_tracing_iters * (1 + p->line_step_iters);
    return trace * (p->coarse_tau > 0.f && p->trace_tier ? 2 : 1);
}

static bool minsdf_share_fits(const nefii_tracer_params *p) {
    return nefii_trace_max_rounds(p) - 1 - trace_rounds(p) >= 6;
}

extern "C" int nefii_trace_max_rounds(const nefii_tracer_params *p) {
    if (!p) return 0;
    const int L = p->bisect_levels >= 1 && p->bisect_levels <= 5 ? p->bisect_levels : 3;
    const int trace = 1 + p->sphere_tracing_iters * (1 + p->line_step_iters);
    return trace + 1 + (p->n_rootfind_steps + L - 1) / L + 1 + 2 +
           (p->coarse_tau > 0.f ? 3 + 3 + 1 + (p->trace_tier ? trace : 0) : 0) + (minsdf_staged(p) ? 1 : 0);
}

extern "C" size_t nefii_trace_workspace_bytes(int64_t n_rays, const nefii_tracer_params *p) {
    if (!p || n_rays <= 0) return 0;
    RayState s;
    size_t bytes = carve(s, nullptr, n_rays, p->n_steps, coarse_cap(p), minsdf_staged(p) ? minsdf_rows(n_rays, p) : 0);
    bytes += align256(sizeof(int) * NCNT * (size_t)nefii_trace_max_rounds(p));
    return bytes;
}

struct TraceJob {
    Params P;
    const nefii_mlp *sdf;
    int precision, rounds, adv_blocks, eval_blocks, eval_blocks_w;
    int pipelined;
    int coarse;
    const void *f8;
    hipStream_t st;
    int32_t *counters;
};

int prepare_job(TraceJob &J, const nefii_mlp *h_sdf, const nefii_tracer_params *h_params, const float *origins,
                const float *dirs, const uint8_t *object_mask, int64_t n_rays, const float *lin_steps,
                const float *minsdf_steps, float *out_points, uint8_t *out_hit, float *out_dists, void *workspace,
                size_t workspace_bytes, int32_t *counters, bool reset, void *stream, const void *cells, int grid_n) {
    if (!h_sdf || !h_params || !origins || !dirs || !object_mask || !lin_steps || !out_points || !out_hit ||
        !out_dists || !workspace)
        return NEFII_E_ARG;
    if (n_rays <= 0 || n_rays >= (1ll << 29)) return NEFII_E_SHAPE;
    if (h_params->training && !minsdf_steps) return NEFII_E_ARG;
    const int levels = h_params->bisect_levels >= 1 && h_params->bisect_levels <= 5 ? h_params->bisect_levels : 3;
    if (h_params->bisect_levels < 0 || h_params->bisect_levels > 5) return NEFII_E_ARG;
    if (h_params->n_steps < (1 << levels) || h_params->sphere_tracing_iters > 250 || h_params->line_step_iters > 15 ||
        h_params->n_rootfind_steps > 250)
        return NEFII_E_SHAPE;
    if (h_params->sphere_tracing_iters < 0 || h_params->line_step_iters < 0 || h_params->n_rootfind_steps < 0)
        return NEFII_E_SHAPE;
    if (!sdf_net_ok(h_sdf)) return NEFII_E_UNSUPPORTED;
    if (workspace_bytes < nefii_trace_workspace_bytes(n_rays, h_params)) return NEFII_E_SHAPE;
    if (h_params->precision < 0 || h_params->precision > 2) return NEFII_E_ARG;
    if (h_params->precision >= 1)
        for (int l = 0; l < h_sdf->n_layers; ++l)
            if (!h_sdf->layer[l].w_f16x3) return NEFII_E_ARG;
    J.sdf = h_sdf;
    J.st = (hipStream_t)stream;
    J.precision = h_params->precision;
    J.rounds = nefii_trace_max_rounds(h_params);
    J.counters = counters;
    Params &P = J.P;
    P.p = *h_params;
    P.n = n_rays;
    P.o = origins;
    P.d = dirs;
    P.obj = object_mask;
    P.lin = lin_steps;
    P.steps = minsdf_steps ? minsdf_steps : lin_steps;
    if (!minsdf_steps) P.p.minsdf_group = 0;
    P.out_pts = out_points;
    P.out_dist = out_dists;
    P.out_hit = out_hit;
    J.pipelined = h_params->precision == 2 ? fits16p(h_sdf) : 0;
    if (h_params->split_fp8 < 0 || h_params->split_fp8 > 1) return NEFII_E_ARG;
    J.f8 = (h_params->split_fp8 && J.pipelined == 4 && nefii_sdf_fp8corr_supported(h_sdf))
               ? (const void *)((const char *)h_sdf->w_stream + stream_bytes_1to4(h_sdf)) : nullptr;
    J.coarse = h_params->coarse_tau > 0.f && J.pipelined && nefii_sdf_coarse_supported(h_sdf) &&
               n_rays < (1ll << 25) && h_params->n_steps <= 128;
    if (h_params->coarse_tau < 0.f || h_params->coarse_tau > 1.f) return NEFII_E_ARG;
    P.tau = J.coarse ? h_params->coarse_tau : 0.f;
    P.cap = coarse_cap(h_params);
    P.chunk = 0;
    P.chunk_gate = 1e30f;
    P.window = 0;
    P.tier_band = 0.f;
    P.tier_gate = 0.f;
    if (h_params->trace_tier < 0 || h_params->trace_tier > 1 || h_params->tier_kappa < 0.f || h_params->tier_gate < 0.f)
        return NEFII_E_ARG;
    if (J.coarse && h_params->trace_tier) {
        const float kappa = h_params->tier_kappa > 0.f ? h_params->tier_kappa : 2.f;
        const float band = kappa * P.tau, least = P.tau + 2.f * fabsf(h_params->sdf_threshold);
        P.tier_band = band > least ? band : least;
        P.tier_gate = (h_params->tier_gate > 0.f ? h_params->tier_gate : 4.f) * P.tau;
    }
    if (J.coarse && h_params->n_steps >= 16) {
        P.window = env_int("NEFII_SAMPLER_WINDOW", 2 | (n_rays >= 32768 ? 1 : 0)) & 3;
    }
    if (J.coarse) {
        const int c = env_int("NEFII_SAMPLER_CHUNK", 6);
        P.chunk = (c >= 2 && c <= 31 && c <= P.cap && c < h_params->n_steps) ? c : 0;
        P.chunk_gate = env_float("NEFII_SAMPLER_CHUNK_GATE", 1.0f);
    }
    if (h_params->minsdf_lipschitz < 0.f || h_params->minsdf_lipschitz > 1e6f) return NEFII_E_ARG;
    const bool staged = J.coarse && minsdf_staged(h_params);
    P.lip = staged ? h_params->minsdf_lipschitz : 0.f;
    P.share = staged && h_params->training && minsdf_share_fits(h_params) && env_int("NEFII_MINSDF_SHARE", 1) != 0;
    static const int stage_bracket = env_int("NEFII_BRACKET_STAGED", 1) != 0;
    P.stage_bracket = stage_bracket;
    if (h_params->unread_misses < 0 || h_params->unread_misses > 1) return NEFII_E_ARG;
    P.miss_argmin = !(h_params->unread_misses && !h_params->training);
    if (cells && (grid_n < 1 || grid_n > NEFII_BOUND_GRID_MAX)) return NEFII_E_SHAPE;
    P.cells = staged ? (const unsigned *)cells : nullptr;
    P.grid_n = grid_n;
    P.grid_inv_h = (float)((double)grid_n / (2.0 * (double)h_params->object_bounding_sphere));
    const int64_t step_rows = minsdf_staged(h_params) ? minsdf_rows(n_rays, &P.p) : 0;
    size_t off = carve(P.s, (char *)workspace, n_rays, h_params->n_steps, P.cap, step_rows);
    P.counters = (int *)((char *)workspace + off);
    P.levels = levels;
    P.tri_nodes = (1 << levels) - 1;
    if (reset) {
        hipError_t e = hipMemsetAsync(P.counters, 0, sizeof(int) * NCNT * J.rounds, J.st);
        if (e != hipSuccess) return (int)e;
        e = hipMemsetAsync(P.s.flags, 0, sizeof(int) * n_rays, J.st);
        if (e != hipSuccess) return (int)e;
        if (staged && h_params->training) {
            hipLaunchKernelGGL(minsdf_order_kernel, dim3((int)minsdf_rows(n_rays, &P.p)), dim3(128), 0, J.st, P);
            HIP_CHECK_LAUNCH();
        }
    }
    J.adv_blocks = (int)((n_rays + 255) / 256);
    const int64_t max_q = n_rays * (int64_t)h_params->n_steps;
    const int64_t max_tiles = (max_q + TILE - 1) / TILE;
    J.eval_blocks = (int)(max_tiles < 1024 ? max_tiles : 1024);
    const int64_t max_tiles_w = (max_q + TILE_W - 1) / TILE_W;
    static const int eval_grid = env_int("NEFII_EVAL_GRID", 0);
    const int grid_cap = eval_grid > 0 ? eval_grid : 2048;
    J.eval_blocks_w = (int)(max_tiles_w < grid_cap ? max_tiles_w : grid_cap);
    return 0;
}

int launch_round(const TraceJob &J, int r, bool profile) {
    hipStream_t st = J.st;
    hipLaunchKernelGGL(advance_kernel, dim3(J.adv_blocks), dim3(256), 0, st, J.P, r);
    HIP_CHECK_LAUNCH();
    if (r + 1 < J.rounds) {
        hipEvent_t e0 = nullptr, e1 = nullptr;
        if (profile) {
            e0 = prof_event();
            e1 = prof_event();
            (void)hipEventRecord(e0, st);
        }
        const int64_t small_tiles = (J.P.n * 2 + 31) / 32 < 256 ? (J.P.n * 2 + 31) / 32 : 256;
        const dim3 big_grid(J.eval_blocks_w), small_grid((int)(small_tiles < 1 ? 1 : small_tiles));
        auto pair = [&](auto big, auto small, int block, const auto &...args) -> int {
            hipLaunchKernelGGL(big, big_grid, dim3(block), 0, st, args...);
            HIP_CHECK_LAUNCH();
            hipLaunchKernelGGL(small, small_grid, dim3(block), 0, st, args...);
            return 0;
        };
        int rc = 0;
        const bool split = J.precision == 2, q_layout = J.sdf->reserved == 1;
        if (split && J.pipelined == 2)
            rc = pair(eval_kernel16q<6, 2>, eval_kernel16q<2, 2>, 512, J.P, *J.sdf, r);
        else if (split && J.pipelined && q_layout && J.f8)
            rc = pair(eval_kernel16f<4>, eval_kernel16f<2>, 512, J.P, *J.sdf, r, J.f8);
        else if (split && J.pipelined && q_layout && J.P.n <= 1024)
            rc = pair(eval_kernel16q<4, 4>, eval_kernel16q<2, 4, true>, 512, J.P, *J.sdf, r);
        else if (split && J.pipelined && q_layout)
            rc = pair(eval_kernel16q<4, 4>, eval_kernel16q<2, 4>, 512, J.P, *J.sdf, r);
        else if (split && J.pipelined)
            rc = pair(eval_kernel16p<P16W, 2>, eval_kernel16p<P16W, 1>, 64 * P16W, J.P, *J.sdf, r);
        else if (split)
            hipLaunchKernelGGL(eval_kernel16w, big_grid, dim3(WG_W), 0, st, J.P, *J.sdf, r);
        else if (J.precision == 1)
            hipLaunchKernelGGL(eval_kernel16, dim3(J.eval_blocks), dim3(WG), 0, st, J.P, *J.sdf, r);
        else
            hipLaunchKernelGGL(eval_kernel, dim3(J.eval_blocks), dim3(WG), 0, st, J.P, *J.sdf, r);
        if (rc) return rc;
        HIP_CHECK_LAUNCH();
        if (J.coarse) {
            const int ft = J.pipelined == 2 ? 2 : 4, rows = coarse_rows(ft);
            const int64_t t = (J.P.n * (int64_t)(4 * coarse_window(J.P.p.n_steps) + 2) + rows - 1) / rows;
            const dim3 grid((int)(t < J.eval_blocks_w ? t : J.eval_blocks_w));
            NEFII_COARSE_LAUNCH(eval_kernel16s, eval_kernel16d, ft, grid, st, J.P, *J.sdf, r);
            HIP_CHECK_LAUNCH();
        }
        if (profile) (void)hipEventRecord(e1, st);
    }
    return 0;
}

int finish_job(const TraceJob &J) {
    if (J.counters) {
        hipError_t e = hipMemcpyAsync(J.counters, J.P.counters, sizeof(int) * NCNT * J.rounds, hipMemcpyDeviceToDevice, J.st);
        if (e != hipSuccess) return (int)e;
    }
    return 0;
}

extern "C" int nefii_trace_rays_rounds_grid(const nefii_mlp *h_sdf, const nefii_tracer_params *h_params,
                                            const float *origins, const float *dirs, const uint8_t *object_mask,
                                            int64_t n_rays, const float *lin_steps, const float *minsdf_steps,
                                            float *out_points, uint8_t *out_hit, float *out_dists, void *workspace,
                                            size_t workspace_bytes, int32_t *counters, int round_begin, int round_end,
                                            const void *cells, int G, void *stream) {
    if (n_rays == 0 && h_sdf && h_params) return 0;
    TraceJob J;
    int rc = prepare_job(J, h_sdf, h_params, origins, dirs, object_mask, n_rays, lin_steps, minsdf_steps, out_points,
                         out_hit, out_dists, workspace, workspace_bytes, counters, round_begin == 0, stream, cells, G);
    if (rc) return rc;
    if (round_end <= 0 || round_end > J.rounds) round_end = J.rounds;
    if (round_begin < 0 || round_begin >= round_end) return NEFII_E_ARG;
    if (g_prof.on) {
        if (!g_prof.t0) {
            (void)hipEventCreate(&g_prof.t0);
            (void)hipEventCreate(&g_prof.t1);
        }
        (void)hipEventRecord(g_prof.t0, J.st);
    }
    for (int r = round_begin; r < round_end; ++r) {
        rc = launch_round(J, r, g_prof.on);
        if (rc) return rc;
    }
    if (g_prof.on) {
        (void)hipEventRecord(g_prof.t1, J.st);
        g_prof.have_span = true;
    }
    return finish_job(J);
}

extern "C" int nefii_trace_rays_rounds(const nefii_mlp *h_sdf, const nefii_tracer_params *h_params,
                                       const float *origins, const float *dirs, const uint8_t *object_mask,
                                       int64_t n_rays, const float *lin_steps, const float *minsdf_steps,
                                       float *out_points, uint8_t *out_hit, float *out_dists, void *workspace,
                                       size_t workspace_bytes, int32_t *counters, int round_begin, int round_end,
                                       void *stream) {
    return nefii_trace_rays_rounds_grid(h_sdf, h_params, origins, dirs, object_mask, n_rays, lin_steps, minsdf_steps, out_points,
                                        out_hit, out_dists, workspace, workspace_bytes, counters, round_begin, round_end, nullptr,
                                        0, stream);
}

extern "C" int nefii_trace_rays_groups_grid(const nefii_mlp *h_sdf, const nefii_tracer_params *h_params,
                                            const float *origins, const float *dirs, const uint8_t *object_mask,
                                            int n_groups, const int64_t *group_begin, const float *lin_steps,
                                            const float *minsdf_steps, float *out_points, uint8_t *out_hit,
                                            float *out_dists, void *const *workspaces, const size_t *workspace_bytes,
                                            int32_t *counters, int round_begin, int round_end, const void *cells, int G,
                                            void *const *streams) {
    if (n_groups < 1 || n_groups > 16 || !group_begin || !workspaces || !workspace_bytes || !streams) return NEFII_E_ARG;
    if (!h_params) return NEFII_E_ARG;
    TraceJob J[16];
    const int rounds = nefii_trace_max_rounds(h_params);
    if (round_end <= 0 || round_end > rounds) round_end = rounds;
    if (round_begin < 0 || round_begin >= round_end) return NEFII_E_ARG;
    for (int g = 0; g < n_groups; ++g) {
        const int64_t lo = group_begin[g], n = group_begin[g + 1] - lo;
        if (lo < 0 || n <= 0) return NEFII_E_ARG;
        int rc = prepare_job(J[g], h_sdf, h_params, origins + 3 * lo, dirs + 3 * lo, object_mask + lo, n, lin_steps,
                             minsdf_steps, out_points + 3 * lo, out_hit + lo, out_dists + lo, workspaces[g],
                             workspace_bytes[g], counters ? counters + (size_t)g * rounds * NCNT : nullptr,
                             round_begin == 0, streams[g], cells, G);
        if (rc) return rc;
    }
    for (int r = round_begin; r < round_end; ++r)
        for (int g = 0; g < n_groups; ++g) {
            int rc = launch_round(J[g], r, false);
            if (rc) return rc;
        }
    for (int g = 0; g < n_groups; ++g) {
        int rc = finish_job(J[g]);
        if (rc) return rc;
    }
    return 0;
}

extern "C" int nefii_trace_rays_groups(const nefii_mlp *h_sdf, const nefii_tracer_params *h_params,
                                       const float *origins, const float *dirs, const uint8_t *object_mask,
                                       int n_groups, const int64_t *group_begin, const float *lin_steps,
                                       const float *minsdf_steps, float *out_points, uint8_t *out_hit,
                                       float *out_dists, void *const *workspaces, const size_t *workspace_bytes,
                                       int32_t *counters, int round_begin, int round_end, void *const *streams) {
    return nefii_trace_rays_groups_grid(h_sdf, h_params, origins, dirs, object_mask, n_groups, group_begin, lin_steps,
                                        minsdf_steps, out_points, out_hit, out_dists, workspaces, workspace_bytes, counters,
                                        round_begin, round_end, nullptr, 0, streams);
}

extern "C" int nefii_trace_rays(const nefii_mlp *h_sdf, const nefii_tracer_params *h_params, const float *origins,
                                const float *dirs, const uint8_t *object_mask, int64_t n_rays, const float *lin_steps,
                                const float *minsdf_steps, float *out_points, uint8_t *out_hit, float *out_dists,
                                void *workspace, size_t workspace_bytes, int32_t *counters, void *stream) {
    return nefii_trace_rays_rounds(h_sdf, h_params, origins, dirs, object_mask, n_rays, lin_steps, minsdf_steps,
                                   out_points, out_hit, out_dists, workspace, workspace_bytes, counters, 0, 0, stream);
}

__global__ void camera_rays_kernel(const float *__restrict__ uv, const float *__restrict__ pose,
                                   const float *__restrict__ K, int batch, int64_t samples, float *__restrict__ dirs,
                                   float *__restrict__ origins) {
    const int64_t total = (int64_t)batch * samples;
    for (int64_t i = (int64_t)blockIdx.x * blockDim.x + threadIdx.x; i < total; i += (int64_t)gridDim.x * blockDim.x) {
        const int b = (int)(i / samples);
        const float *Kb = K + b * 16, *Pb = pose + b * 16;
        const float fx = Kb[0], sk = Kb[1], cx = Kb[2], fy = Kb[5], cy = Kb[6];
        const float u = uv[i * 2], v = uv[i * 2 + 1];
        const float x = __fdiv_rn(fsub(fadd(fsub(u, cx), __fdiv_rn(fmul(cy, sk), fy)), __fdiv_rn(fmul(sk, v), fy)), fx);
        const float y = __fdiv_rn(fsub(v, cy), fy);
        float w[3];
        for (int c = 0; c < 3; ++c) {
            const float wc = fadd(fadd(fadd(fmul(Pb[c * 4], x), fmul(Pb[c * 4 + 1], y)), Pb[c * 4 + 2]), Pb[c * 4 + 3]);
            w[c] = fsub(wc, Pb[c * 4 + 3]);
        }
        const float nrm = fmaxf(sqrtf(fadd(fadd(fmul(w[0], w[0]), fmul(w[1], w[1])), fmul(w[2], w[2]))), 1e-12f);
        for (int c = 0; c < 3; ++c) {
            dirs[i * 3 + c] = __fdiv_rn(w[c], nrm);
            origins[i * 3 + c] = Pb[c * 4 + 3];
        }
    }
}

extern "C" int nefii_camera_rays(const float *uv, const float *pose, const float *intrinsics, int batch,
                                 int64_t samples, float *out_dirs, float *out_origins, void *stream) {
    if (!uv || !pose || !intrinsics || !out_dirs || !out_origins) return NEFII_E_ARG;
    const int64_t total = (int64_t)batch * samples;
    if (total <= 0) return 0;
    int blocks = (int)((total + 255) / 256 < 2048 ? (total + 255) / 256 : 2048);
    hipLaunchKernelGGL(camera_rays_kernel, dim3(blocks), dim3(256), 0, (hipStream_t)stream, uv, pose, intrinsics, batch,
                       samples, out_dirs, out_origins);
    HIP_CHECK_LAUNCH();
    return 0;
}
```

### nefii_amd/model/implicit_differentiable_renderer.py

```python
import math
import os

import numpy as np
import torch
import torch.nn as nn

from .. import ops
from ..utils import rend_util
from .ray_tracing import RayTracing
from .sample_network import SampleNetwork
from .sg_envmap_material import EnvmapMaterialNetwork
from .sg_render import render_with_sg


def _params_version(module):
    return tuple((p.data_ptr(), p._version) for p in _plist(module))


_plist = ops.param_list


class ImplicitNetwork(nn.Module):

    def __init__(self, feature_vector_size, d_in, d_out, dims, geometric_init=True, bias=1.0, skip_in=(),
                 weight_norm=True, multires=0, use_last_as_f=False):
        super().__init__()
        if use_last_as_f:
            assert feature_vector_size == dims[-1]
        assert d_in == 3
        self.feature_vector_size = feature_vector_size
        self.cfg = dict(d_in=d_in, d_out=d_out, dims=list(dims), skip_in=list(skip_in), multires=multires,
                        use_last_as_f=use_last_as_f)
        self.specs, self.enc = ops.sdf_specs(self.cfg, feature_vector_size)
        self.num_layers = len(self.specs) + 1
        self.skip_in = skip_in
        self.use_last_as_f = use_last_as_f
        self.weight_norm = weight_norm
        d0 = self.specs[0].k_in
        for l, s in enumerate(self.specs):
            lin = nn.Linear(s.k_in, s.n_out)
            if geometric_init:
                if l == len(self.specs) - 1:
                    nn.init.normal_(lin.weight, mean=np.sqrt(np.pi) / np.sqrt(s.k_in), std=0.0001)
                    nn.init.constant_(lin.bias, -bias)
                else:
                    nn.init.constant_(lin.bias, 0.0)
                    nn.init.normal_(lin.weight, 0.0, np.sqrt(2) / np.sqrt(s.n_out))
                    if multires > 0 and l == 0:
                        nn.init.constant_(lin.weight[:, 3:], 0.0)
                    elif multires > 0 and l in skip_in:
                        nn.init.constant_(lin.weight[:, -(d0 - 3):], 0.0)
            if weight_norm:
                lin = nn.utils.weight_norm(lin)
            setattr(self, 'lin' + str(l), lin)
        self._pm = None
        self._pm_version = None
        self._pm_fit = None
        self._tau = None
        self.coarse_audit_max = 0.0
        self.coarse_audit_events = []
        self._lip = None
        self._grid = None

    def coarse_tau(self, radius=1.0):
        pm = self.packed(f16x3=True)
        if self._tau is None or self._tau[0] != self._pm_version or self._tau[1] != radius:
            self._tau = (self._pm_version, radius, ops.calibrate_coarse_tau(pm, radius))
        return self._tau[2]

    def minsdf_lipschitz(self, radius=1.0):
        self.packed(f16x3=True)
        if self._lip is None or self._lip[0] != self._pm_version or self._lip[1] != radius:
            with torch.no_grad():
                self._lip = (self._pm_version, radius, ops.calibrate_lipschitz(self.gradient, _plist(self)[0].device, radius))
        return self._lip[2]

    def bound_grid(self, radius=1.0, G=None):
        pm = self.packed(f16x3=True)
        tau = self.coarse_tau(radius)
        if not tau > 0.0 or not self.minsdf_lipschitz(radius) > 0.0:
            return None
        G = int(G or ops.BOUND_GRID_SIZE)
        key = (self._pm_version, radius, tau, G)
        if self._grid is None or self._grid[:4] != key:
            self._grid = key + (ops.build_bound_grid(pm, radius, tau, G),)
        return self._grid[4]

    def note_lipschitz_audit(self, violation, lip_used):
        if violation <= 0.0 or lip_used <= 0.0 or self._lip is None or self._lip[0] != self._pm_version or self._lip[2] <= 0.0:
            return
        import warnings
        warnings.warn('staged min-SDF search of the tracer disabled for this network: a depth lay %.3e below the lower bound '
                      'its claimed Lipschitz constant %.3f gives' % (violation, lip_used))
        self._lip = (self._pm_version, self._lip[1], 0.0)
        self._grid = None
        self.coarse_audit_events.append(('lipschitz_disabled', float(violation), float(lip_used)))

    def note_coarse_audit(self, observed, tau_used, radius=1.0):
        self.coarse_audit_max = max(self.coarse_audit_max, float(observed))
        if self._tau is None or self._tau[0] != self._pm_version or self._tau[2] <= 0.0 or tau_used <= 0.0:
            return
        tau = self._tau[2]
        if observed > tau_used:
            import warnings
            warnings.warn('coarse pass of the tracer disabled for this network: a refined sample differed from its '
                          'single-pass value by %.3e, above the claimed bound %.3e' % (observed, tau_used))
            self._tau = (self._pm_version, self._tau[1], 0.0)
            self.coarse_audit_events.append(('disabled', float(observed), float(tau_used)))
        elif observed * 2.0 > tau:
            self._tau = (self._pm_version, self._tau[1], ops.COARSE_TAU_SAFETY * float(observed))
            self.coarse_audit_events.append(('recalibrated', float(observed), float(tau_used)))

    def effective_weights(self):
        ws, bs = [], []
        for l in range(len(self.specs)):
            lin = getattr(self, 'lin' + str(l))
            if self.weight_norm:
                ws.append(torch._weight_norm(lin.weight_v, lin.weight_g, 0))
            else:
                ws.append(lin.weight)
            bs.append(lin.bias)
        return ws, bs

    def packed(self, f16x3=False):
        ver = _params_version(self)
        dev = _plist(self)[0].device
        if self._pm is None or self._pm.device != dev or (f16x3 and not self._pm.f16x3):
            self._pm = ops.PackedMLP(self.specs, ops.ACT_SOFTPLUS100, ops.HEAD_NONE, self.enc, 0, dev, f16x3=f16x3)
            self._pm_version = None
        if self._pm_version != ver:
            with torch.no_grad():
                ws, bs = self.effective_weights()
                self._pm.pack(ws, bs)
            self._pm_version = ver
        return self._pm

    def _check_frozen(self):
        if torch.is_grad_enabled() and any(p.requires_grad for p in _plist(self)):
            raise NotImplementedError(
                'nefii_amd: differentiating through the SDF network (trainable geometry) is outside the Step-2 '
                'hot path; call IDRNetwork.freeze_geometry() as every shipped Step-2 script does')

    def _trainable(self):
        return torch.is_grad_enabled() and any(p.requires_grad for p in _plist(self))

    def forward(self, input, compute_grad=False):
        x = ops._f32(input)
        if self._trainable():
            ws, bs = self.effective_weights()
            pm = ops.PackedMLP(self.specs, ops.ACT_SOFTPLUS100, ops.HEAD_NONE, self.enc, 0, x.device) \
                if self._pm_fit is None or self._pm_fit.device != x.device else self._pm_fit
            self._pm_fit = pm
            if self.use_last_as_f:
                out, hidden = ops.FusedMLPHiddenFn.apply(pm, x.detach(), *ws, *bs)
                return torch.cat([out, hidden], dim=-1)
            return ops.FusedMLPFn.apply(pm, x.detach(), None, None, None, *ws, *bs)
        out, hidden, _ = ops.mlp_forward(self.packed(), x, None, None, None, want_hidden=self.use_last_as_f)
        if self.use_last_as_f:
            out = torch.cat([out, hidden], dim=-1)
        return out

    def gradient(self, x, no_grad=False):
        self._check_frozen()
        _, _, g = ops.sdf_value_grad(self.packed(), ops._f32(x))
        return g.unsqueeze(1)

    def value_feature_gradient(self, x):
        self._check_frozen()
        out, hidden, g = ops.sdf_value_grad(self.packed(), ops._f32(x), want_feat=self.use_last_as_f)
        if self.use_last_as_f:
            feat = hidden
        elif self.feature_vector_size > 0:
            feat = out[:, 1:].contiguous()
        else:
            feat = None
        return out[:, :1], feat, g


class RenderingNetwork(nn.Module):

    def __init__(self, feature_vector_size, mode, d_in, d_out, dims, weight_norm=True, weight_init=False,
                 multires_view=0, multires_xyz=0, normalize_output=True, clip_output=False, clip_method='relu'):
        super().__init__()
        self.feature_vector_size = feature_vector_size
        self.mode = mode
        self.normalize_output = normalize_output
        self.clip_output = clip_output
        self.clip_method = clip_method
        self.weight_norm = weight_norm
        self.cfg = dict(mode=mode, d_in=d_in, d_out=d_out, dims=list(dims), multires_view=multires_view,
                        multires_xyz=multires_xyz, normalize_output=normalize_output, clip_output=clip_output,
                        clip_method=clip_method)
        self.specs, self.enc, self.head = ops.radiance_specs(self.cfg, feature_vector_size)
        self.num_layers = len(self.specs) + 1
        lins = []
        for l, s in enumerate(self.specs):
            lins.append(nn.Linear(s.k_in, s.n_out))
        if weight_init:
            for lin in lins[:-1]:
                nn.init.kaiming_uniform_(lin.weight, mode='fan_in', nonlinearity='relu')
                nn.init.constant_(lin.bias, 0.0)
            nn.init.constant_(lins[-1].bias, 0.0)
            if normalize_output:
                nn.init.xavier_uniform_(lins[-1].weight, gain=nn.init.calculate_gain('tanh'))
            elif clip_method == 'relu':
                nn.init.kaiming_uniform_(lins[-1].weight, mode='fan_in', nonlinearity='relu')
        for l, lin in enumerate(lins):
            if weight_norm:
                lin = nn.utils.weight_norm(lin)
            setattr(self, 'lin' + str(l), lin)
        self._pm = None
        self.outputs_detached = False
        self._packed_for = None

    def packed(self, device):
        half = ops.mlp_precision() if ops.mlp_precision() in ('f16', 'f16x3') else False
        if self._pm is None or self._pm.device != device or self._pm.half != half:
            self._pm = ops.PackedMLP(self.specs, ops.ACT_RELU, self.head, self.enc, self.feature_vector_size, device,
                                     half=half)
        return self._pm

    def _effective_weights(self):
        ws, bs = [], []
        for l in range(len(self.specs)):
            lin = getattr(self, 'lin' + str(l))
            ws.append(torch._weight_norm(lin.weight_v, lin.weight_g, 0) if self.weight_norm else lin.weight)
            bs.append(lin.bias)
        return ws, bs

    def forward(self, points, normals, view_dirs, feature_vectors=None):
        p, n, v = ops._f32(points), ops._f32(normals), ops._f32(view_dirs)
        if self.mode == 'idr':
            a, b, c = p, v, n
        elif self.mode == 'no_view_dir':
            a, b, c = p, n, None
        else:
            a, b, c = p, v, None
        feat = ops._f32(feature_vectors) if self.feature_vector_size > 0 else None
        pm = self.packed(p.device)
        if self.outputs_detached or not torch.is_grad_enabled() or not any(q.requires_grad for q in _plist(self)):
            key = (_params_version(self), id(pm))
            with torch.no_grad():
                if self._packed_for != key:
                    pm.pack(*self._effective_weights())
                    self._packed_for = key
                return ops.mlp_forward(pm, a, b, c, feat, want_stash=False)[0]
        self._packed_for = None
        ws, bs = self._effective_weights()
        return ops.FusedMLPFn.apply(pm, a, b, c, feat, *ws, *bs)


class IDRNetwork(nn.Module):
    def __init__(self, conf):
        super().__init__()
        self.feature_vector_size = conf.get_int('feature_vector_size')
        self.correct_normal = conf.get_bool('correct_normal', default=False)
        if self.correct_normal:
            raise NotImplementedError('correct_normal is broken in the reference (attribute shadows the method)')
        self.implicit_network = ImplicitNetwork(self.feature_vector_size, **conf.get_config('implicit_network'))
        self.rendering_network = RenderingNetwork(self.feature_vector_size, **conf.get_config('rendering_network'))
        self.envmap_material_network = EnvmapMaterialNetwork(correct_normal=False,
                                                             feature_vector_size=self.feature_vector_size,
                                                             **conf.get_config('envmap_material_network'))
        self.ray_tracer = RayTracing(**conf.get_config('ray_tracer'))
        self.ray_tracer.bind(self.implicit_network)
        self.sample_network = SampleNetwork()
        self.object_bounding_sphere = conf.get_float('ray_tracer.object_bounding_sphere')
        self.render_type = conf.get_string('render_type', default='sg')
        self.rgb_render = self.get_rgb_render(self.render_type)
        self.fast_multi_ray = conf.get_bool('fast_multi_ray', default=False)
        if self.fast_multi_ray:
            raise NotImplementedError('fast_multi_ray (off in every shipped conf)')
        self.render_background = conf.get_bool('render_background', default=False)
        self.state_freeze_geo = False
        self.state_freeze_idr = False
        self.state_freeze_env_mat = False
        self.secondary_miss_search = os.environ.get('NEFII_SECONDARY_MISS_SEARCH', '0') == '1'
        self.envmap_light = None
        self.envmap_indirect = 'mlp'

    def set_envmap_light(self, light, indirect='mlp'):
        from .path_tracing_render import INDIRECT_MODES
        if indirect not in INDIRECT_MODES:
            raise ValueError('indirect is one of %s, not %r' % (', '.join(INDIRECT_MODES), indirect))
        if light is not None and self.render_type not in ('pt_render_indirect_mlp', 'pt_render_indirect_mlp_memsave'):
            raise ValueError('a map light needs render_type pt_render_indirect_mlp(_memsave), this model has %r'
                             % self.render_type)
        self.envmap_light = light
        self.envmap_indirect = indirect if light is not None else 'mlp'

    def freeze_geometry(self):
        for p in self.implicit_network.parameters():
            p.requires_grad = False
        self.state_freeze_geo = True

    def unfreeze_geometry(self):
        for p in self.implicit_network.parameters():
            p.requires_grad = True
        self.state_freeze_geo = False

    def freeze_idr(self):
        self.freeze_geometry()
        for p in self.rendering_network.parameters():
            p.requires_grad = False
        self.state_freeze_idr = True

    def unfreeze_idr(self):
        self.unfreeze_geometry()
        for p in self.rendering_network.parameters():
            p.requires_grad = True
        self.state_freeze_idr = False

    def freeze_decompose_render(self):
        for p in self.envmap_material_network.parameters():
            p.requires_grad = False
        self.state_freeze_env_mat = True

    def unfreeze_decompose_render(self):
        for p in self.envmap_material_network.parameters():
            p.requires_grad = True
        self.state_freeze_env_mat = False

    def train(self, mode: bool = True):
        nn.Module.train(self, mode)
        if self.state_freeze_idr:
            self.rendering_network.eval()
        if self.state_freeze_geo:
            self.implicit_network.eval()
        if self.state_freeze_env_mat:
            self.envmap_material_network.eval()
        return self

    def forward(self, input, with_point=False):
        if self.envmap_light is not None and self.training:
            raise RuntimeError('a map light (set_envmap_light) is for rendering: call eval() first, or set it to None')
        if not with_point:
            return self.forward_with_uv(input)
        return self.forward_with_point(input)

    def forward_with_uv(self, input):
        if self.training and not self.state_freeze_geo:
            from . import trainable_geometry
            return trainable_geometry.forward_with_uv(self, input)
        ctx = self.trace_head(input)
        idx = torch.nonzero(ctx['network_object_mask']).flatten()
        return self.shade_tail(ctx, idx)

    def trace_head(self, input):
        return self.attach_surface(self.trace_points(input))

    @staticmethod
    def _batch_rays(input):
        uv, object_mask = input['uv'], input['object_mask'].reshape(-1)
        shape = None
        if uv.dim() == 4:
            B, S, R, _ = uv.shape
            shape = (B, S, R)
            uv = uv.reshape(B, S * R, 2)
            object_mask = object_mask.reshape(B, S, 1).expand(B, S, R).reshape(-1)
        ray_dirs, cam_loc = rend_util.get_camera_params(uv, input['pose'], input['intrinsics'])
        return ray_dirs, cam_loc, object_mask, shape

    def trace_points(self, input):
        if self.training and not self.state_freeze_geo:
            raise NotImplementedError('the kernel path needs frozen geometry (freeze_geometry()); forward() routes '
                                      'trainable geometry to model/trainable_geometry.py')
        ray_dirs, cam_loc, object_mask, shape = self._batch_rays(input)
        with torch.no_grad():
            points, network_object_mask, dists = self.ray_tracer(sdf=self.implicit_network, cam_loc=cam_loc,
                                                                 object_mask=object_mask, ray_directions=ray_dirs)
        return {'points': points, 'network_object_mask': network_object_mask, 'object_mask': object_mask,
                'ray_dirs': ray_dirs.reshape(-1, 3), 'multi': shape}

    def trace_points_group(self, inputs):
        if self.training and not self.state_freeze_geo:
            raise NotImplementedError('the kernel path needs frozen geometry (freeze_geometry())')
        dirs, cams, masks, shapes = [], [], [], []
        for input in inputs:
            ray_dirs, cam_loc, object_mask, shape = self._batch_rays(input)
            if ray_dirs.shape[0] != 1 or (dirs and ray_dirs.shape != dirs[0].shape):
                raise ValueError('trace_points_group: one image per batch, equal ray counts')
            dirs.append(ray_dirs), cams.append(cam_loc), masks.append(object_mask), shapes.append(shape)
        rt = self.ray_tracer
        rt.steps_per_batch = True
        try:
            with torch.no_grad():
                points, hit, dists = rt(sdf=self.implicit_network, cam_loc=torch.cat(cams), object_mask=torch.cat(masks),
                                        ray_directions=torch.cat(dirs))
        finally:
# ... 243 lines not shown
```

### nefii_amd/model/ray_tracing.py

```python
import contextlib
import os

import torch
import torch.nn as nn

from .. import ops


class RayTracing(nn.Module):
    def __init__(self, object_bounding_sphere=1.0, sdf_threshold=5.0e-5, line_search_step=0.5, line_step_iters=1,
                 sphere_tracing_iters=10, n_steps=100, n_rootfind_steps=8, trace_tier=None):
        super().__init__()
        self.object_bounding_sphere = object_bounding_sphere
        self.sdf_threshold = sdf_threshold
        self.sphere_tracing_iters = sphere_tracing_iters
        self.line_step_iters = line_step_iters
        self.line_search_step = line_search_step
        self.n_steps = n_steps
        self.n_rootfind_steps = n_rootfind_steps
        self._net = None
        self.precision = os.environ.get('NEFII_TRACER_PRECISION', 'f16x3w')
        self._lin = None
        self.last_counters = None
        self.counter_sum = None
        self.collect_counters = False
        self.minsdf_steps_override = None
        self._calls = 0
        self.bisect_levels = int(os.environ.get('NEFII_BISECT_LEVELS', '0'))
        self.concurrent = False
        self.adaptive_rounds = True
        self._rounds_state = {}
        self.stream_groups = int(os.environ.get('NEFII_TRACER_GROUPS', '0'))
        self.skip_min_sdf_search = False
        self.draw_when_skipped = False
        self.miss_search = True
        self.steps_per_batch = False
        self.deferred_checks = None
        self.coarse = os.environ.get('NEFII_TRACER_COARSE', '1') != '0'
        self.coarse_tau_override = None
        self.coarse_cap = int(os.environ.get('NEFII_TRACER_COARSE_CAP', '0'))
        self.coarse_min_rays = int(os.environ.get('NEFII_COARSE_MIN_RAYS', '1024'))
        env = os.environ.get('NEFII_TRACE_TIER')
        self.trace_tier = (bool(trace_tier) if trace_tier is not None else self.TIER_DEFAULT) if env is None or env == '' \
            else env != '0'
        self.tier_kappa = float(os.environ.get('NEFII_TIER_KAPPA', '0'))
        self.tier_gate = float(os.environ.get('NEFII_TIER_GATE', '0'))
        self.minsdf_staged = os.environ.get('NEFII_MINSDF_STAGED', '1') != '0'
        self.bracket_staged_eval = os.environ.get('NEFII_BRACKET_STAGED_EVAL', '0') == '1'
        self.bound_grid = os.environ.get('NEFII_BOUND_GRID', '1') != '0'
        self.bound_grid_size = int(os.environ.get('NEFII_BOUND_GRID_SIZE', '0'))
        self.minsdf_lipschitz_override = None
        self.split_fp8 = os.environ.get('NEFII_SPLIT_FP8', '0') == '1'
        self.retraced_calls = 0

    @staticmethod
    def auto_levels(n_rays, concurrent=False):
        if n_rays >= 131072:
            return 1
        if concurrent or n_rays > 16384:
            return 3
        return 5

    @staticmethod
    def small_round_for(n_rays, concurrent):
        env = os.environ.get('NEFII_SMALL_ROUND')
        if env:
            return int(env)
        return 4096 if concurrent and n_rays > 1024 else 0

    TIER_DEFAULT = False

    def tier_for(self, n_rays=None):
        return bool(self.trace_tier)

    @contextlib.contextmanager
    def enqueued_ahead(self, checks):
        self.deferred_checks, self.concurrent = checks, True
        try:
            yield
        finally:
            self.deferred_checks, self.concurrent = None, False

    def bind(self, implicit_network):
        object.__setattr__(self, '_net', implicit_network)

    def _cfg(self):
        return dict(object_bounding_sphere=self.object_bounding_sphere, sdf_threshold=self.sdf_threshold,
                    line_search_step=self.line_search_step, line_step_iters=self.line_step_iters,
                    sphere_tracing_iters=self.sphere_tracing_iters, n_steps=self.n_steps,
                    n_rootfind_steps=self.n_rootfind_steps)

    def _bounds(self, net, n_rays, frozen, training=True):
        tau, lip, audit, grid = 0.0, 0.0, None, None
        if self.coarse and self.precision == 'f16x3w' and (n_rays > self.coarse_min_rays or self.tier_for()) and \
                (frozen or self.coarse_tau_override is not None):
            tau = self.coarse_tau_override if self.coarse_tau_override is not None else \
                net.coarse_tau(self.object_bounding_sphere)
            use_grid = not training and not self.bracket_staged_eval and self.bound_grid and frozen and \
                self.coarse_tau_override is None and self.minsdf_lipschitz_override is None
            if tau > 0 and self.minsdf_staged and (training or self.bracket_staged_eval or use_grid):
                lip = self.minsdf_lipschitz_override if self.minsdf_lipschitz_override is not None else \
                    net.minsdf_lipschitz(self.object_bounding_sphere)
                if use_grid:
                    grid = net.bound_grid(self.object_bounding_sphere, self.bound_grid_size) if lip > 0 else None
                    if grid is None:
                        lip = 0.0
            if tau > 0 and (self.coarse_tau_override is None or (lip > 0 and self.minsdf_lipschitz_override is None)):
                radius, used, lip_used = self.object_bounding_sphere, tau, lip
                check_tau, check_lip = self.coarse_tau_override is None, self.minsdf_lipschitz_override is None

                def audit(v, lip_violation=0.0):
                    if check_tau:
                        net.note_coarse_audit(v, used, radius)
                    if check_lip and not v > used:
                        net.note_lipschitz_audit(lip_violation, lip_used)
        return tau, lip, audit, grid

    def forward(self, sdf, cam_loc, object_mask, ray_directions):
        net = sdf if hasattr(sdf, 'packed') else self._net
        if net is None:
            raise RuntimeError('RayTracing: no ImplicitNetwork bound; call ray_tracer.bind(implicit_network) or '
                               'pass the network as `sdf`')
        B, S, _ = ray_directions.shape
        dirs = ops._f32(ray_directions).reshape(-1, 3)
        origins = ops._f32(cam_loc).unsqueeze(1).expand(B, S, 3).reshape(-1, 3).contiguous()
        dev = dirs.device
        if self._lin is None or self._lin.device != dev or self._lin.numel() != self.n_steps:
            self._lin = torch.linspace(0, 1, steps=self.n_steps).to(dev)
        steps = None
        training = self.training and not self.skip_min_sdf_search and self.miss_search
        if self.training and not self.skip_min_sdf_search and not self.miss_search and \
                isinstance(self.minsdf_steps_override, (list, tuple)):
            self._calls += 1
        if self.training and self.skip_min_sdf_search and self.draw_when_skipped and self.miss_search and \
                self.minsdf_steps_override is None:
            for _ in range(B if (self.steps_per_batch and B > 1) else 1):
                torch.empty(self.n_steps).uniform_(0.0, 1.0)
        group = 0
        if training:
            rows = B if (self.steps_per_batch and B > 1) else 1
            drawn = []
            for _ in range(rows):
                if self.minsdf_steps_override is not None:
                    ov = self.minsdf_steps_override
                    if isinstance(ov, (list, tuple)):
                        ov = ov[self._calls % len(ov)]
                        self._calls += 1
                    drawn.append(ov.reshape(-1))
                else:
                    drawn.append(torch.empty(self.n_steps).uniform_(0.0, 1.0))
            steps = drawn[0] if rows == 1 else torch.stack([d.cpu() for d in drawn])
            if steps.device.type == 'cpu' and dev.type == 'cuda':
                steps = steps.contiguous().pin_memory().to(dev, non_blocking=True)
            else:
                steps = steps.to(dev).contiguous()
            group = S if rows > 1 else 0
        n_rays = dirs.shape[0]
        levels = self.bisect_levels or self.auto_levels(n_rays, self.concurrent)
        frozen = not any(p.requires_grad for p in ops.param_list(net))
        state = None
        if self.adaptive_rounds:
            import math
            state = self._rounds_state.setdefault((training, int(math.log2(n_rays + 1))), ops.TraceRounds())
        deferred = self.deferred_checks
        for attempt in range(3):
            seen = len(net.coarse_audit_events)
            tau, lip, audit, grid = self._bounds(net, n_rays, frozen, training)
            params = ops.make_tracer_params(self._cfg(), training, self.precision, levels, coarse_tau=tau,
                                            coarse_cap=self.coarse_cap, minsdf_group=group,
                                            small_round=self.small_round_for(n_rays, self.concurrent),
                                            trace_tier=self.tier_for(), tier_kappa=self.tier_kappa,
                                            tier_gate=self.tier_gate, minsdf_lipschitz=lip,
                                            unread_misses=0 if self.miss_search else 1, split_fp8=self.split_fp8)
            res = ops.trace_rays(net.packed(f16x3=self.precision.startswith('f16x3')), params, origins, dirs,
                                 object_mask.reshape(-1), self._lin, steps, want_counters=self.collect_counters,
                                 rounds_state=state,
                                 groups=1 if group else (self.stream_groups or 1),
                                 deferred=deferred,
                                 audit=audit, bound_grid=grid)
            if deferred is not None or audit is None or not any(
                    kind in ('disabled', 'lipschitz_disabled') for kind, _, _ in net.coarse_audit_events[seen:]):
                break
            self.retraced_calls += 1
        if self.collect_counters:
            self.last_counters = res[3]
            cur = res[3]
            if self.counter_sum is not None and self.counter_sum.shape[0] != cur.shape[0]:
                n = max(self.counter_sum.shape[0], cur.shape[0])
                pad = lambda t: torch.cat([t, t.new_zeros(n - t.shape[0], t.shape[1])]) if t.shape[0] < n else t
                self.counter_sum, cur = pad(self.counter_sum), pad(cur)
            self.counter_sum = cur.clone() if self.counter_sum is None else ops.sum_counters(self.counter_sum, cur)
        return res[0], res[1], res[2]
```

### nefii_amd/ops/tracer.py

```python
import ctypes

import torch

from .. import _lib
from .._lib import TracerParams
from ._call import _f32, _ptr, call
from ._call import nbytes as _nbytes


def algorithmic_evals(counters, n_steps):
    c = counters.long()
    return (c[..., _lib.CNT_SINGLES] + c[..., _lib.CNT_COARSE_SINGLES] - c[..., _lib.CNT_REPEATS]
            + c[..., _lib.CNT_SEARCHES] * n_steps + c[..., _lib.CNT_BISECT_USED])


def executed_evals(counters, n_steps, tri_nodes=None):
    c = counters.long()
    split = c[..., _lib.CNT_SINGLES] + c[..., _lib.CNT_DENSE_ROWS] * n_steps + c[..., _lib.CNT_BISECT_EVALS] + c[..., _lib.CNT_REFINED]
    coarse = (c[..., _lib.CNT_COARSE_WINDOWS] * ((n_steps + 3) // 4) + c[..., _lib.CNT_COARSE_SINGLES]
              + c[..., _lib.CNT_COARSE_SAMPLES])
    return split, coarse


PRECISIONS = {'f32': 0, 'f16x3': 1, 'f16x3w': 2}


def make_tracer_params(cfg, training, precision='f32', bisect_levels=3, coarse_tau=0.0, coarse_cap=0, minsdf_group=0,
                       small_round=0, trace_tier=0, tier_kappa=0.0, tier_gate=0.0, minsdf_lipschitz=0.0, unread_misses=0,
                       split_fp8=0):
    p = TracerParams()
    p.split_fp8 = 1 if split_fp8 else 0
    p.unread_misses = 1 if unread_misses else 0
    p.minsdf_lipschitz = float(minsdf_lipschitz) if coarse_tau > 0.0 else 0.0
    p.trace_tier = 1 if (trace_tier and coarse_tau > 0.0) else 0
    p.tier_kappa = float(tier_kappa)
    p.tier_gate = float(tier_gate)
    p.minsdf_group = int(minsdf_group)
    p.small_round = int(small_round)
    p.precision = PRECISIONS[precision]
    p.bisect_levels = bisect_levels
    p.coarse_tau = float(coarse_tau)
    p.coarse_cap = int(coarse_cap)
    p.object_bounding_sphere = cfg.get('object_bounding_sphere', 1.0)
    p.sdf_threshold = cfg.get('sdf_threshold', 5.0e-5)
    p.line_search_step = cfg.get('line_search_step', 0.5)
    p.line_step_iters = cfg.get('line_step_iters', 1)
    p.sphere_tracing_iters = cfg.get('sphere_tracing_iters', 10)
    p.n_steps = cfg.get('n_steps', 100)
    p.n_rootfind_steps = cfg.get('n_rootfind_steps', 8)
    p.training = 1 if training else 0
    return p


class TraceRounds:

    def __init__(self):
        self.guess = None


_TRACE_STREAMS = {}
_WORK = _lib.CNT_WORK


_SIDE_STREAMS = {}


def side_stream(dev):
    key = torch.device(dev).index if torch.device(dev).index is not None else torch.cuda.current_device()
    st = _SIDE_STREAMS.get(key)
    if st is None:
        st = _SIDE_STREAMS[key] = torch.cuda.Stream(device=key)
    return st


def _trace_streams(dev, n):
    pool = _TRACE_STREAMS.setdefault(dev, [])
    while len(pool) < n:
        pool.append(torch.cuda.Stream(device=dev))
    return pool[:n]


def sum_counters(a, b=None):
    if b is None:
        out = a.sum(dim=0)
        for col in _lib.CNT_MAXIMA:
            out[..., col] = a[..., col].max(dim=0).values
        return out
    out = a + b
    for col in _lib.CNT_MAXIMA:
        out[..., col] = torch.maximum(a[..., col], b[..., col])
    return out


def _lip_audit_of(host_counters):
    col = host_counters[..., _lib.CNT_LIP_AUDIT].contiguous().view(torch.float32)
    return float(col.max()) if col.numel() else 0.0


def _audit_of(host_counters):
    col = host_counters[..., _lib.CNT_TAU_AUDIT].contiguous().view(torch.float32)
    return float(col.max()) if col.numel() else 0.0


def _chunks_with_work(host, guess):
    if guess >= host.shape[1]:
        return []
    return [g for g in range(host.shape[0]) if int(host[g, guess - 1, _WORK].sum()) > 0]


def _next_guess(host):
    busy = torch.nonzero(host[:, :, _WORK].sum(dim=(0, 2))).flatten()
    return (int(busy[-1]) if busy.numel() else 0) + 3


BOUND_GRID_SIZE = 256
BOUND_GRID_L_FLOOR = 1.0
BOUND_GRID_SAFETY = 1.5


def build_bound_grid(pm_sdf, radius, tau, G=BOUND_GRID_SIZE, l_floor=BOUND_GRID_L_FLOOR, safety=BOUND_GRID_SAFETY):
    cells = torch.empty(G, G, G, device=pm_sdf.device, dtype=torch.int32)
    ws = torch.empty(_nbytes('nefii_sdf_bound_grid_workspace_bytes', G), device=pm_sdf.device, dtype=torch.uint8)
    call('nefii_sdf_bound_grid_build', ctypes.byref(pm_sdf.struct), G, float(radius), float(tau), float(l_floor), float(safety),
         _ptr(cells), _ptr(ws))
    return cells


def trace_rays(pm_sdf, params, origins, dirs, object_mask, lin_steps, minsdf_steps=None, want_counters=False,
               rounds_state=None, groups=1, deferred=None, audit=None, keep_workspace=None, bound_grid=None):
    lib = _lib.lib()
    n = origins.shape[0]
    dev = origins.device
    pts = torch.empty(n, 3, device=dev, dtype=torch.float32)
    hit = torch.empty(n, device=dev, dtype=torch.uint8)
    dist = torch.empty(n, device=dev, dtype=torch.float32)
    rounds = lib.nefii_trace_max_rounds(ctypes.byref(params))
    if audit is not None and rounds_state is None and torch.cuda.is_current_stream_capturing():
        audit = None
    need_cnt = want_counters or rounds_state is not None or audit is not None
    groups = max(1, min(int(groups), n // 64)) if n > 0 else 1
    counters = torch.zeros(groups, rounds, _lib.TRACE_COUNTERS, device=dev, dtype=torch.int32) if need_cnt else None
    if n > 0:
        om = object_mask.to(torch.uint8).contiguous()
        per = -(-n // groups)
        per = -(-per // 64) * 64
        bounds = [(g * per, min(n, (g + 1) * per)) for g in range(groups) if g * per < n]
        cur = torch.cuda.current_stream(dev)
        streams = [cur] if len(bounds) == 1 else _trace_streams(dev, len(bounds))
        if len(bounds) > 1:
            start = cur.record_event()
        work = []
        for g, (lo, hi) in enumerate(bounds):
            with torch.cuda.stream(streams[g]):
                if len(bounds) > 1:
                    streams[g].wait_event(start)
                nbytes = lib.nefii_trace_workspace_bytes(hi - lo, ctypes.byref(params))
                work.append((torch.empty(nbytes, device=dev, dtype=torch.uint8), nbytes))

        if keep_workspace is not None:
            keep_workspace.extend((w, lo, hi - lo) for (w, _), (lo, hi) in zip(work, bounds))
        G = len(bounds)
        begin = (ctypes.c_int64 * (G + 1))(*([lo for lo, _ in bounds] + [n]))
        ws_ptrs = (ctypes.c_void_p * G)(*[w.data_ptr() for w, _ in work])
        ws_bytes = (ctypes.c_size_t * G)(*[b for _, b in work])
        st_ptrs = (ctypes.c_void_p * G)(*[st.cuda_stream for st in streams])
        cells, cells_n = (_ptr(bound_grid), bound_grid.shape[0]) if bound_grid is not None else (None, 0)

        def run(sel, r0, r1):
            if len(sel) == G and G > 1:
                b_, w_, wb_, s_, c_ = begin, ws_ptrs, ws_bytes, st_ptrs, counters
                call('nefii_trace_rays_groups_grid', ctypes.byref(pm_sdf.struct), ctypes.byref(params), _ptr(origins), _ptr(dirs),
                     _ptr(om), G, b_, _ptr(lin_steps), _ptr(minsdf_steps), _ptr(pts), _ptr(hit), _ptr(dist), w_, wb_,
                     _ptr(c_) if c_ is not None else None, r0, r1, cells, cells_n, stream=s_)
                return
            for g in sel:
                lo, hi = bounds[g]
                ws, nbytes = work[g]
                call('nefii_trace_rays_rounds_grid', ctypes.byref(pm_sdf.struct), ctypes.byref(params), _ptr(origins[lo:hi]),
                     _ptr(dirs[lo:hi]), _ptr(om[lo:hi]), hi - lo, _ptr(lin_steps), _ptr(minsdf_steps), _ptr(pts[lo:hi]),
                     _ptr(hit[lo:hi]), _ptr(dist[lo:hi]), _ptr(ws), nbytes, _ptr(counters[g]) if counters is not None else None,
                     r0, r1, cells, cells_n, stream=streams[g].cuda_stream)

        def join():
            for st in streams:
                if st is not cur:
                    cur.wait_event(st.record_event())

        def pinned_counters():
            ahead = torch.empty(counters.shape, dtype=counters.dtype, pin_memory=True)
            return ahead.copy_(counters, non_blocking=True)

        def tell(host):
            if audit is not None:
                audit(_audit_of(host), _lip_audit_of(host))

        everyone = list(range(G))
        if rounds_state is None:
            run(everyone, 0, 0)
            join()
            if audit is not None:
                if deferred is not None:
                    deferred.append(lambda ahead=pinned_counters(): tell(ahead))
                else:
                    tell(counters.cpu())
        else:
            guess = rounds if rounds_state.guess is None else max(2, min(rounds, rounds_state.guess))
            run(everyone, 0, guess)
            join()

            def settle(host, wait):
                again = _chunks_with_work(host, guess)
                if again:
                    run(again, guess, 0)
                    wait()
                    host = counters.cpu()
                rounds_state.guess = _next_guess(host)
                tell(host)
                return again

            def sync_streams():
                for st in streams:
                    st.synchronize()

            if deferred is not None:
                ahead = pinned_counters()
                deferred.append(lambda: (pts, hit.bool(), dist) if settle(ahead, sync_streams) else None)
            else:
                settle(counters.cpu(), join)
    if want_counters:
        return pts, hit.bool(), dist, sum_counters(counters)
    return pts, hit.bool(), dist


def trace_iterations(kept):
    out = []
    for ws, _lo, n in kept:
        stride = (4 * n + 255) // 256 * 256
        begin = _lib.TRACE_WS_FLOAT_ARRAYS * stride
        flags = ws[begin:begin + 4 * n].view(torch.int32)
        out.append((flags >> _lib.TRACE_ITER_SHIFT) & 0xF)
    return torch.cat(out)


def camera_rays(uv, pose, intrinsics):
    B, S, _ = uv.shape
    dirs = torch.empty(B, S, 3, device=uv.device, dtype=torch.float32)
    orig = torch.empty(B, S, 3, device=uv.device, dtype=torch.float32)
    uv_c, pose_c, k_c = _f32(uv), _f32(pose), _f32(intrinsics)
    call('nefii_camera_rays', _ptr(uv_c), _ptr(pose_c), _ptr(k_c), B, S, _ptr(dirs), _ptr(orig))
    return dirs, orig
```

Before: 2.099 million rays/s.

## Tighten bound-grid brackets with per-vertex half SDF values and cell Lipschitz

Extends the SDF bound grid with fp16 SDF values at grid vertices and a per-cell directional Lipschitz estimate. During bracket setup, samples not already excluded get a tighter lower and upper bound from the eight cell corners plus Lipschitz reach. The goal is to rule out more samples and rays before dense SDF evaluation. In exchange it adds extra memory reads and arithmetic per sample, a new build kernel, and a larger grid. It is on by default through an environment flag.

New measurement: 2.146 million rays/s, median of 6. +2.3%, better.

```diff
diff --git a/include/nefii_amd.h b/include/nefii_amd.h
--- a/include/nefii_amd.h
+++ b/include/nefii_amd.h
@@ -200,6 +200,24 @@
                                  void *const *workspaces, const size_t *workspace_bytes, int32_t *counters,
                                  int round_begin, int round_end, const void *cells, int G, void *const *streams);
 
+int nefii_sdf_bound_grid_build_vertices(const nefii_mlp *h_sdf, int G, float radius, float tau, float L_floor, float safety,
+                                        void *out_cells, void *out_vertex_g, void *out_cell_l, void *workspace, void *stream);
+int nefii_trace_rays_rounds_grid_vertices(const nefii_mlp *h_sdf, const nefii_tracer_params *h_params,
+                                          const float *origins, const float *dirs, const uint8_t *object_mask, int64_t n_rays,
+                                          const float *lin_steps, const float *minsdf_steps,
+                                          float *out_points, uint8_t *out_hit, float *out_dists,
+                                          void *workspace, size_t workspace_bytes, int32_t *counters,
+                                          int round_begin, int round_end, const void *cells, int G,
+                                          const void *vertex_g, const void *cell_l, void *stream);
+int nefii_trace_rays_groups_grid_vertices(const nefii_mlp *h_sdf, const nefii_tracer_params *h_params,
+                                          const float *origins, const float *dirs, const uint8_t *object_mask,
+                                          int n_groups, const int64_t *group_begin,
+                                          const float *lin_steps, const float *minsdf_steps,
+                                          float *out_points, uint8_t *out_hit, float *out_dists,
+                                          void *const *workspaces, const size_t *workspace_bytes, int32_t *counters,
+                                          int round_begin, int round_end, const void *cells, int G,
+                                          const void *vertex_g, const void *cell_l, void *const *streams);
+
 int nefii_trace_profile_enable(int on);
 int nefii_trace_profile_read(double *h_eval_ms, int *h_n_eval, double *h_span_ms);
 int nefii_trace_profile_launches(float *h_ms, int cap);
diff --git a/nefii_amd/_lib.py b/nefii_amd/_lib.py
--- a/nefii_amd/_lib.py
+++ b/nefii_amd/_lib.py
@@ -138,6 +138,11 @@
                                          ctypes.c_size_t, P, I, I, P, I, P]),
     'nefii_trace_rays_groups_grid': (I, [ctypes.POINTER(Mlp), ctypes.POINTER(TracerParams), P, P, P, I, P, P, P, P, P, P, P, P,
                                          P, I, I, P, I, P]),
+    'nefii_sdf_bound_grid_build_vertices': (I, [ctypes.POINTER(Mlp), I, F, F, F, F, P, P, P, P, P]),
+    'nefii_trace_rays_rounds_grid_vertices': (I, [ctypes.POINTER(Mlp), ctypes.POINTER(TracerParams), P, P, P, I64, P, P, P, P, P,
+                                                  P, ctypes.c_size_t, P, I, I, P, I, P, P, P]),
+    'nefii_trace_rays_groups_grid_vertices': (I, [ctypes.POINTER(Mlp), ctypes.POINTER(TracerParams), P, P, P, I, P, P, P, P, P,
+                                                  P, P, P, P, I, I, P, I, P, P, P]),
     'nefii_trace_profile_enable': (I, [I]),
     'nefii_trace_profile_read': (I, [ctypes.POINTER(ctypes.c_double), ctypes.POINTER(I), ctypes.POINTER(ctypes.c_double)]),
     'nefii_trace_profile_launches': (I, [ctypes.POINTER(ctypes.c_float), I]),
diff --git a/nefii_amd/csrc/nefii_tracer.hip b/nefii_amd/csrc/nefii_tracer.hip
--- a/nefii_amd/csrc/nefii_tracer.hip
+++ b/nefii_amd/csrc/nefii_tracer.hip
@@ -87,6 +87,8 @@
     const unsigned *cells;
     int grid_n;
     float grid_inv_h;
+    const unsigned short *vert_g, *cell_l;
+    float grid_h;
     RayState s;
 };
 
@@ -317,6 +319,45 @@
     return true;
 }
 
+__device__ __forceinline__ bool grid_corner_bounds(const Params &P, int64_t r, float t, float &lo, float &hi) {
+    const float rad = P.p.object_bounding_sphere, g = (float)P.grid_n;
+    const float ox = P.o[r * 3], oy = P.o[r * 3 + 1], oz = P.o[r * 3 + 2];
+    const float dx = P.d[r * 3], dy = P.d[r * 3 + 1], dz = P.d[r * 3 + 2];
+    const float px = fadd(ox, fmul(t, dx)), py = fadd(oy, fmul(t, dy)), pz = fadd(oz, fmul(t, dz));
+    const float fx = fmul(fadd(px, rad), P.grid_inv_h), fy = fmul(fadd(py, rad), P.grid_inv_h), fz = fmul(fadd(pz, rad), P.grid_inv_h);
+    lo = -__builtin_inff(), hi = __builtin_inff();
+    if (!(fx >= 0.f && fx < g && fy >= 0.f && fy < g && fz >= 0.f && fz < g)) return false;
+    const int ci = (int)fx, cj = (int)fy, ck = (int)fz;
+    const size_t V = (size_t)P.grid_n + 1;
+    const float L = (float)__builtin_bit_cast(_Float16, P.cell_l[((size_t)ci * P.grid_n + (size_t)cj) * P.grid_n + (size_t)ck]);
+    unsigned short gc[8];
+#pragma unroll
+    for (int c = 0; c < 4; ++c) {
+        const unsigned short *row = P.vert_g + ((size_t)(ci + (c >> 1)) * V + (size_t)(cj + (c & 1))) * V + (size_t)ck;
+        gc[2 * c] = row[0];
+        gc[2 * c + 1] = row[1];
+    }
+    float ex2[2], ey2[2], ez2[2];
+#pragma unroll
+    for (int a = 0; a < 2; ++a) {
+        const float ex = fsub(px, fadd(-rad, fmul((float)(ci + a), P.grid_h)));
+        const float ey = fsub(py, fadd(-rad, fmul((float)(cj + a), P.grid_h)));
+        const float ez = fsub(pz, fadd(-rad, fmul((float)(ck + a), P.grid_h)));
+        ex2[a] = fmul(ex, ex), ey2[a] = fmul(ey, ey), ez2[a] = fmul(ez, ez);
+    }
+#pragma unroll
+    for (int c = 0; c < 8; ++c) {
+        const float v = (float)__builtin_bit_cast(_Float16, gc[c]);
+        const float dist = fadd(sqrtf(fadd(fadd(ex2[c >> 2], ey2[(c >> 1) & 1]), ez2[c & 1])), 1e-6f);
+        const float reach = fadd(fmul(L, dist), fadd(fmul(fabsf(v), 0x1p-11f), 0x1p-25f));
+        lo = fmaxf(lo, fsub(v, reach));
+        hi = fminf(hi, fadd(v, reach));
+    }
+    lo = fsub(lo, P.tau);
+    hi = fadd(hi, P.tau);
+    return true;
+}
+
 __device__ __forceinline__ void begin_grid_bracket(const Params &P, int64_t r, int round, int from, int &fl, Emit &e) {
     const int ns = P.p.n_steps;
     float *v = P.s.big + (size_t)r * ns;
@@ -335,10 +376,29 @@
         if (i == 0) lo0 = lo;
         if (i >= from) v[i] = lo;
     }
-    const bool front_only = obj && j1 < ns && lo0 > 0.f;
-    const bool sign_only = front_only || !P.miss_argmin;
-    const float lim = sign_only ? 0.f : fmaxf(0.f, fadd(U, P.tau));
-    const int last = front_only ? j1 : ns - 1;
+    bool front_only = obj && j1 < ns && lo0 > 0.f;
+    bool sign_only = front_only || !P.miss_argmin;
+    float lim = sign_only ? 0.f : fmaxf(0.f, fadd(U, P.tau));
+    int last = front_only ? j1 : ns - 1;
+    if (P.vert_g) {
+        for (int i = from; i <= last; ++i) {
+            const float lb = v[i];
+            if (fsub(lb, 1e-6f) > lim) continue;
+            float lo, hi;
+            if (!grid_corner_bounds(P, r, fadd(a, fmul(P.lin[i], rng)), lo, hi)) continue;
+            v[i] = fmaxf(lb, lo);
+            if (i == 0) lo0 = v[i];
+            U = fminf(U, hi);
+            if (hi < -P.tau && i < j1) {
+                j1 = i;
+                if (obj && lo0 > 0.f) break;
+            }
+        }
+        front_only = obj && j1 < ns && lo0 > 0.f;
+        sign_only = front_only || !P.miss_argmin;
+        lim = sign_only ? 0.f : fmaxf(0.f, fadd(U, P.tau));
+        last = front_only ? j1 : ns - 1;
+    }
     int k = 0, n_near = 0, probe = -1;
     unsigned probe_h = ~0u;
     for (int i = from; i < ns; ++i) {
@@ -377,10 +437,18 @@
     const float *v = P.s.big + (size_t)r * ns;
     const float a = P.s.t_s[r], rng = fsub(P.s.t_e[r], a);
     float worst = 0.f;
+    int n_corner = 0;
     for (int i = 0; i < ns; ++i) {
         if (!(v[i] < __builtin_inff())) continue;
         float lo, hi;
-        if (!grid_bounds(P, r, fadd(a, fmul(P.lin[i], rng)), lo, hi)) continue;
+        const float t = fadd(a, fmul(P.lin[i], rng));
+        if (!grid_bounds(P, r, t, lo, hi)) continue;
+        if (P.vert_g && n_corner < CREF_CAP) {
+            float lo_c, hi_c;
+            grid_corner_bounds(P, r, t, lo_c, hi_c);
+            lo = fmaxf(lo, lo_c), hi = fminf(hi, hi_c);
+            ++n_corner;
+        }
         worst = fmaxf(worst, fmaxf(fsub(fsub(lo, P.tau), v[i]), fsub(v[i], fadd(hi, P.tau))));
     }
     if (worst > 0.f) atomicMax(P.counters + round * NCNT + NEFII_CNT_LIP_AUDIT, __float_as_int(worst));
@@ -2391,28 +2459,46 @@
 }
 
 __global__ __launch_bounds__(256) void grid_cells_kernel(int G, float h, float tau, float l_floor, float safety,
-                                                         const float *__restrict__ g, unsigned *__restrict__ cells) {
+                                                         const float *__restrict__ g, unsigned *__restrict__ cells,
+                                                         unsigned short *__restrict__ cell_l) {
     const int V = G + 1;
     const int64_t n = (int64_t)G * G * G;
     const float reach = (float)((double)h * 0.8660254037844386);
     for (int64_t c = (int64_t)blockIdx.x * blockDim.x + threadIdx.x; c < n; c += (int64_t)gridDim.x * blockDim.x) {
         const int k = (int)(c % G), j = (int)((c / G) % G), i = (int)(c / ((int64_t)G * G));
         auto at = [&](int a, int b, int d) { return g[((int64_t)a * V + b) * V + d]; };
-        float lo = __builtin_inff(), hi = -__builtin_inff(), slope = 0.f;
+        float lo = __builtin_inff(), hi = -__builtin_inff();
+        float ux = -__builtin_inff(), uy = ux, uz = ux, dx = __builtin_inff(), dy = dx, dz = dx;
+        auto edge = [&](float &u, float &d, float next, float here) {
+            const float s = __fdiv_rn(fsub(next, here), h);
+            u = fmaxf(u, s), d = fminf(d, s);
+        };
         for (int a = i - 1; a <= i + 2; ++a)
             for (int b = j - 1; b <= j + 2; ++b)
                 for (int d = k - 1; d <= k + 2; ++d) {
                     if (a < 0 || a > G || b < 0 || b > G || d < 0 || d > G) continue;
                     const float v = at(a, b, d);
                     if (a >= i && a <= i + 1 && b >= j && b <= j + 1 && d >= k && d <= k + 1) lo = fminf(lo, v), hi = fmaxf(hi, v);
-                    if (a < i + 2 && a < G) slope = fmaxf(slope, __fdiv_rn(fabsf(fsub(at(a + 1, b, d), v)), h));
-                    if (b < j + 2 && b < G) slope = fmaxf(slope, __fdiv_rn(fabsf(fsub(at(a, b + 1, d), v)), h));
-                    if (d < k + 2 && d < G) slope = fmaxf(slope, __fdiv_rn(fabsf(fsub(at(a, b, d + 1), v)), h));
+                    if (a < i + 2 && a < G) edge(ux, dx, at(a + 1, b, d), v);
+                    if (b < j + 2 && b < G) edge(uy, dy, at(a, b + 1, d), v);
+                    if (d < k + 2 && d < G) edge(uz, dz, at(a, b, d + 1), v);
                 }
+        const float sx = fmaxf(fabsf(ux), fabsf(dx)), sy = fmaxf(fabsf(uy), fabsf(dy)), sz = fmaxf(fabsf(uz), fabsf(dz));
+        const float slope = fmaxf(fmaxf(sx, sy), sz);
         const float lcell = fmaxf(fmul(safety, slope), l_floor);
         const float slack = fadd(tau, fmul(lcell, reach));
         cells[c] = (unsigned)half_toward(fsub(lo, slack), false) | ((unsigned)half_toward(fadd(hi, slack), true) << 16);
-    }
+        if (cell_l) {
+            const float mx = fadd(sx, fsub(ux, dx)), my = fadd(sy, fsub(uy, dy)), mz = fadd(sz, fsub(uz, dz));
+            const float norm = sqrtf(fadd(fadd(fmul(mx, mx), fmul(my, my)), fmul(mz, mz)));
+            cell_l[c] = half_toward(fmaxf(fmul(safety, norm), l_floor), true);
+        }
+    }
+}
+
+__global__ __launch_bounds__(256) void grid_vertex_half_kernel(int64_t n, const float *__restrict__ g, unsigned short *__restrict__ out) {
+    for (int64_t q = (int64_t)blockIdx.x * blockDim.x + threadIdx.x; q < n; q += (int64_t)gridDim.x * blockDim.x)
+        out[q] = __builtin_bit_cast(unsigned short, (_Float16)g[q]);
 }
 }
 
@@ -2424,7 +2510,14 @@
 
 extern "C" int nefii_sdf_bound_grid_build(const nefii_mlp *h_sdf, int G, float radius, float tau, float L_floor, float safety,
                                           void *out_cells, void *workspace, void *stream) {
+    return nefii_sdf_bound_grid_build_vertices(h_sdf, G, radius, tau, L_floor, safety, out_cells, nullptr, nullptr, workspace, stream);
+}
+
+extern "C" int nefii_sdf_bound_grid_build_vertices(const nefii_mlp *h_sdf, int G, float radius, float tau, float L_floor,
+                                                   float safety, void *out_cells, void *out_vertex_g, void *out_cell_l,
+                                                   void *workspace, void *stream) {
     if (!h_sdf || !out_cells || !workspace || h_sdf->n_layers < 1 || h_sdf->n_layers > NEFII_MAX_LAYERS) return NEFII_E_ARG;
+    if (!out_vertex_g != !out_cell_l) return NEFII_E_ARG;
     if (!(radius > 0.f && radius < 1e6f) || !(tau >= 0.f && tau < 1e6f) || !(L_floor > 0.f && L_floor < 1e6f) ||
         !(safety > 0.f && safety < 1e6f))
         return NEFII_E_ARG;
@@ -2449,8 +2542,14 @@
     }
     const int64_t n_cells = (int64_t)G * G * G;
     hipLaunchKernelGGL(grid_cells_kernel, dim3((int)((n_cells + 255) / 256 < 4096 ? (n_cells + 255) / 256 : 4096)), dim3(256), 0,
-                       st, G, h, tau, L_floor, safety, (const float *)g, (unsigned *)out_cells);
+                       st, G, h, tau, L_floor, safety, (const float *)g, (unsigned *)out_cells, (unsigned short *)out_cell_l);
     HIP_CHECK_LAUNCH();
+    if (out_vertex_g) {
+        const int64_t n_vert = (int64_t)V * V * V;
+        hipLaunchKernelGGL(grid_vertex_half_kernel, dim3((int)((n_vert + 255) / 256 < 4096 ? (n_vert + 255) / 256 : 4096)), dim3(256),
+                           0, st, n_vert, (const float *)g, (unsigned short *)out_vertex_g);
+        HIP_CHECK_LAUNCH();
+    }
     return 0;
 }
 
@@ -2537,7 +2636,8 @@
 int prepare_job(TraceJob &J, const nefii_mlp *h_sdf, const nefii_tracer_params *h_params, const float *origins,
                 const float *dirs, const uint8_t *object_mask, int64_t n_rays, const float *lin_steps,
                 const float *minsdf_steps, float *out_points, uint8_t *out_hit, float *out_dists, void *workspace,
-                size_t workspace_bytes, int32_t *counters, bool reset, void *stream, const void *cells, int grid_n) {
+                size_t workspace_bytes, int32_t *counters, bool reset, void *stream, const void *cells, int grid_n,
+                const void *vertex_g, const void *cell_l) {
     if (!h_sdf || !h_params || !origins || !dirs || !object_mask || !lin_steps || !out_points || !out_hit ||
         !out_dists || !workspace)
         return NEFII_E_ARG;
@@ -2615,6 +2715,10 @@
     P.cells = staged ? (const unsigned *)cells : nullptr;
     P.grid_n = grid_n;
     P.grid_inv_h = (float)((double)grid_n / (2.0 * (double)h_params->object_bounding_sphere));
+    if (!vertex_g != !cell_l || (vertex_g && !cells)) return NEFII_E_ARG;
+    P.vert_g = P.cells ? (const unsigned short *)vertex_g : nullptr;
+    P.cell_l = P.cells ? (const unsigned short *)cell_l : nullptr;
+    P.grid_h = grid_n > 0 ? (float)(2.0 * (double)h_params->object_bounding_sphere / (double)grid_n) : 0.f;
     const int64_t step_rows = minsdf_staged(h_params) ? minsdf_rows(n_rays, &P.p) : 0;
     size_t off = carve(P.s, (char *)workspace, n_rays, h_params->n_steps, P.cap, step_rows);
     P.counters = (int *)((char *)workspace + off);
@@ -2700,16 +2804,18 @@
     return 0;
 }
 
-extern "C" int nefii_trace_rays_rounds_grid(const nefii_mlp *h_sdf, const nefii_tracer_params *h_params,
-                                            const float *origins, const float *dirs, const uint8_t *object_mask,
-                                            int64_t n_rays, const float *lin_steps, const float *minsdf_steps,
-                                            float *out_points, uint8_t *out_hit, float *out_dists, void *workspace,
-                                            size_t workspace_bytes, int32_t *counters, int round_begin, int round_end,
-                                            const void *cells, int G, void *stream) {
+extern "C" int nefii_trace_rays_rounds_grid_vertices(const nefii_mlp *h_sdf, const nefii_tracer_params *h_params,
+                                                     const float *origins, const float *dirs, const uint8_t *object_mask,
+                                                     int64_t n_rays, const float *lin_steps, const float *minsdf_steps,
+                                                     float *out_points, uint8_t *out_hit, float *out_dists, void *workspace,
+                                                     size_t workspace_bytes, int32_t *counters, int round_begin, int round_end,
+                                                     const void *cells, int G, const void *vertex_g, const void *cell_l,
+                                                     void *stream) {
     if (n_rays == 0 && h_sdf && h_params) return 0;
     TraceJob J;
     int rc = prepare_job(J, h_sdf, h_params, origins, dirs, object_mask, n_rays, lin_steps, minsdf_steps, out_points,
-                         out_hit, out_dists, workspace, workspace_bytes, counters, round_begin == 0, stream, cells, G);
+                         out_hit, out_dists, workspace, workspace_bytes, counters, round_begin == 0, stream, cells, G, vertex_g,
+                         cell_l);
     if (rc) return rc;
     if (round_end <= 0 || round_end > J.rounds) round_end = J.rounds;
     if (round_begin < 0 || round_begin >= round_end) return NEFII_E_ARG;
@@ -2729,6 +2835,17 @@
         g_prof.have_span = true;
     }
     return finish_job(J);
+}
+
+extern "C" int nefii_trace_rays_rounds_grid(const nefii_mlp *h_sdf, const nefii_tracer_params *h_params,
+                                            const float *origins, const float *dirs, const uint8_t *object_mask,
+                                            int64_t n_rays, const float *lin_steps, const float *minsdf_steps,
+                                            float *out_points, uint8_t *out_hit, float *out_dists, void *workspace,
+                                            size_t workspace_bytes, int32_t *counters, int round_begin, int round_end,
+                                            const void *cells, int G, void *stream) {
+    return nefii_trace_rays_rounds_grid_vertices(h_sdf, h_params, origins, dirs, object_mask, n_rays, lin_steps, minsdf_steps,
+                                                 out_points, out_hit, out_dists, workspace, workspace_bytes, counters, round_begin,
+                                                 round_end, cells, G, nullptr, nullptr, stream);
 }
 
 extern "C" int nefii_trace_rays_rounds(const nefii_mlp *h_sdf, const nefii_tracer_params *h_params,
@@ -2742,13 +2859,13 @@
                                         0, stream);
 }
 
-extern "C" int nefii_trace_rays_groups_grid(const nefii_mlp *h_sdf, const nefii_tracer_params *h_params,
-                                            const float *origins, const float *dirs, const uint8_t *object_mask,
-                                            int n_groups, const int64_t *group_begin, const float *lin_steps,
-                                            const float *minsdf_steps, float *out_points, uint8_t *out_hit,
-                                            float *out_dists, void *const *workspaces, const size_t *workspace_bytes,
-                                            int32_t *counters, int round_begin, int round_end, const void *cells, int G,
-                                            void *const *streams) {
+extern "C" int nefii_trace_rays_groups_grid_vertices(const nefii_mlp *h_sdf, const nefii_tracer_params *h_params,
+                                                     const float *origins, const float *dirs, const uint8_t *object_mask,
+                                                     int n_groups, const int64_t *group_begin, const float *lin_steps,
+                                                     const float *minsdf_steps, float *out_points, uint8_t *out_hit,
+                                                     float *out_dists, void *const *workspaces, const size_t *workspace_bytes,
+                                                     int32_t *counters, int round_begin, int round_end, const void *cells, int G,
+                                                     const void *vertex_g, const void *cell_l, void *const *streams) {
     if (n_groups < 1 || n_groups > 16 || !group_begin || !workspaces || !workspace_bytes || !streams) return NEFII_E_ARG;
     if (!h_params) return NEFII_E_ARG;
     TraceJob J[16];
@@ -2761,7 +2878,7 @@
         int rc = prepare_job(J[g], h_sdf, h_params, origins + 3 * lo, dirs + 3 * lo, object_mask + lo, n, lin_steps,
                              minsdf_steps, out_points + 3 * lo, out_hit + lo, out_dists + lo, workspaces[g],
                              workspace_bytes[g], counters ? counters + (size_t)g * rounds * NCNT : nullptr,
-                             round_begin == 0, streams[g], cells, G);
+                             round_begin == 0, streams[g], cells, G, vertex_g, cell_l);
         if (rc) return rc;
     }
     for (int r = round_begin; r < round_end; ++r)
@@ -2774,6 +2891,18 @@
         if (rc) return rc;
     }
     return 0;
+}
+
+extern "C" int nefii_trace_rays_groups_grid(const nefii_mlp *h_sdf, const nefii_tracer_params *h_params,
+                                            const float *origins, const float *dirs, const uint8_t *object_mask,
+                                            int n_groups, const int64_t *group_begin, const float *lin_steps,
+                                            const float *minsdf_steps, float *out_points, uint8_t *out_hit,
+                                            float *out_dists, void *const *workspaces, const size_t *workspace_bytes,
+                                            int32_t *counters, int round_begin, int round_end, const void *cells, int G,
+                                            void *const *streams) {
+    return nefii_trace_rays_groups_grid_vertices(h_sdf, h_params, origins, dirs, object_mask, n_groups, group_begin, lin_steps,
+                                                 minsdf_steps, out_points, out_hit, out_dists, workspaces, workspace_bytes,
+                                                 counters, round_begin, round_end, cells, G, nullptr, nullptr, streams);
 }
 
 extern "C" int nefii_trace_rays_groups(const nefii_mlp *h_sdf, const nefii_tracer_params *h_params,
diff --git a/nefii_amd/model/implicit_differentiable_renderer.py b/nefii_amd/model/implicit_differentiable_renderer.py
--- a/nefii_amd/model/implicit_differentiable_renderer.py
+++ b/nefii_amd/model/implicit_differentiable_renderer.py
@@ -75,16 +75,17 @@
                 self._lip = (self._pm_version, radius, ops.calibrate_lipschitz(self.gradient, _plist(self)[0].device, radius))
         return self._lip[2]
 
-    def bound_grid(self, radius=1.0, G=None):
+    def bound_grid(self, radius=1.0, G=None, vertices=False):
         pm = self.packed(f16x3=True)
         tau = self.coarse_tau(radius)
         if not tau > 0.0 or not self.minsdf_lipschitz(radius) > 0.0:
-            return None
+            return (None, None) if vertices else None
         G = int(G or ops.BOUND_GRID_SIZE)
         key = (self._pm_version, radius, tau, G)
-        if self._grid is None or self._grid[:4] != key:
-            self._grid = key + (ops.build_bound_grid(pm, radius, tau, G),)
-        return self._grid[4]
+        if self._grid is None or self._grid[:4] != key or (vertices and self._grid[5] is None):
+            built = ops.build_bound_grid(pm, radius, tau, G, vertices=vertices)
+            self._grid = key + (built if vertices else (built, None))
+        return self._grid[4:6] if vertices else self._grid[4]
 
     def note_lipschitz_audit(self, violation, lip_used):
         if violation <= 0.0 or lip_used <= 0.0 or self._lip is None or self._lip[0] != self._pm_version or self._lip[2] <= 0.0:
diff --git a/nefii_amd/model/ray_tracing.py b/nefii_amd/model/ray_tracing.py
--- a/nefii_amd/model/ray_tracing.py
+++ b/nefii_amd/model/ray_tracing.py
@@ -49,6 +49,7 @@
         self.bracket_staged_eval = os.environ.get('NEFII_BRACKET_STAGED_EVAL', '0') == '1'
         self.bound_grid = os.environ.get('NEFII_BOUND_GRID', '1') != '0'
         self.bound_grid_size = int(os.environ.get('NEFII_BOUND_GRID_SIZE', '0'))
+        self.bound_grid_vertices = os.environ.get('NEFII_BOUND_GRID_VERTICES', '1') != '0'
         self.minsdf_lipschitz_override = None
         self.split_fp8 = os.environ.get('NEFII_SPLIT_FP8', '0') == '1'
         self.retraced_calls = 0
@@ -91,7 +92,7 @@
                     n_rootfind_steps=self.n_rootfind_steps)
 
     def _bounds(self, net, n_rays, frozen, training=True):
-        tau, lip, audit, grid = 0.0, 0.0, None, None
+        tau, lip, audit, grid, verts = 0.0, 0.0, None, None, None
         if self.coarse and self.precision == 'f16x3w' and (n_rays > self.coarse_min_rays or self.tier_for()) and \
                 (frozen or self.coarse_tau_override is not None):
             tau = self.coarse_tau_override if self.coarse_tau_override is not None else \
@@ -102,7 +103,10 @@
                 lip = self.minsdf_lipschitz_override if self.minsdf_lipschitz_override is not None else \
                     net.minsdf_lipschitz(self.object_bounding_sphere)
                 if use_grid:
-                    grid = net.bound_grid(self.object_bounding_sphere, self.bound_grid_size) if lip > 0 else None
+                    if lip > 0 and self.bound_grid_vertices:
+                        grid, verts = net.bound_grid(self.object_bounding_sphere, self.bound_grid_size, vertices=True)
+                    elif lip > 0:
+                        grid = net.bound_grid(self.object_bounding_sphere, self.bound_grid_size)
                     if grid is None:
                         lip = 0.0
             if tau > 0 and (self.coarse_tau_override is None or (lip > 0 and self.minsdf_lipschitz_override is None)):
@@ -114,7 +118,7 @@
                         net.note_coarse_audit(v, used, radius)
                     if check_lip and not v > used:
                         net.note_lipschitz_audit(lip_violation, lip_used)
-        return tau, lip, audit, grid
+        return tau, lip, audit, grid, verts
 
     def forward(self, sdf, cam_loc, object_mask, ray_directions):
         net = sdf if hasattr(sdf, 'packed') else self._net
@@ -165,7 +169,7 @@
         deferred = self.deferred_checks
         for attempt in range(3):
             seen = len(net.coarse_audit_events)
-            tau, lip, audit, grid = self._bounds(net, n_rays, frozen, training)
+            tau, lip, audit, grid, verts = self._bounds(net, n_rays, frozen, training)
             params = ops.make_tracer_params(self._cfg(), training, self.precision, levels, coarse_tau=tau,
                                             coarse_cap=self.coarse_cap, minsdf_group=group,
                                             small_round=self.small_round_for(n_rays, self.concurrent),
@@ -177,7 +181,7 @@
                                  rounds_state=state,
                                  groups=1 if group else (self.stream_groups or 1),
                                  deferred=deferred,
-                                 audit=audit, bound_grid=grid)
+                                 audit=audit, bound_grid=grid, bound_vertices=verts)
             if deferred is not None or audit is None or not any(
                     kind in ('disabled', 'lipschitz_disabled') for kind, _, _ in net.coarse_audit_events[seen:]):
                 break
diff --git a/nefii_amd/ops/tracer.py b/nefii_amd/ops/tracer.py
--- a/nefii_amd/ops/tracer.py
+++ b/nefii_amd/ops/tracer.py
@@ -118,16 +118,25 @@
 BOUND_GRID_SAFETY = 1.5
 
 
-def build_bound_grid(pm_sdf, radius, tau, G=BOUND_GRID_SIZE, l_floor=BOUND_GRID_L_FLOOR, safety=BOUND_GRID_SAFETY):
-    cells = torch.empty(G, G, G, device=pm_sdf.device, dtype=torch.int32)
-    ws = torch.empty(_nbytes('nefii_sdf_bound_grid_workspace_bytes', G), device=pm_sdf.device, dtype=torch.uint8)
-    call('nefii_sdf_bound_grid_build', ctypes.byref(pm_sdf.struct), G, float(radius), float(tau), float(l_floor), float(safety),
-         _ptr(cells), _ptr(ws))
-    return cells
+def build_bound_grid(pm_sdf, radius, tau, G=BOUND_GRID_SIZE, l_floor=BOUND_GRID_L_FLOOR, safety=BOUND_GRID_SAFETY,
+                     vertices=False):
+    dev = pm_sdf.device
+    cells = torch.empty(G, G, G, device=dev, dtype=torch.int32)
+    ws = torch.empty(_nbytes('nefii_sdf_bound_grid_workspace_bytes', G), device=dev, dtype=torch.uint8)
+    if not vertices:
+        call('nefii_sdf_bound_grid_build', ctypes.byref(pm_sdf.struct), G, float(radius), float(tau), float(l_floor), float(safety),
+             _ptr(cells), _ptr(ws))
+        return cells
+    vert_g = torch.empty(G + 1, G + 1, G + 1, device=dev, dtype=torch.float16)
+    cell_l = torch.empty(G, G, G, device=dev, dtype=torch.float16)
+    call('nefii_sdf_bound_grid_build_vertices', ctypes.byref(pm_sdf.struct), G, float(radius), float(tau), float(l_floor),
+         float(safety), _ptr(cells), _ptr(vert_g), _ptr(cell_l), _ptr(ws))
+    return cells, (vert_g, cell_l)
 
 
 def trace_rays(pm_sdf, params, origins, dirs, object_mask, lin_steps, minsdf_steps=None, want_counters=False,
-               rounds_state=None, groups=1, deferred=None, audit=None, keep_workspace=None, bound_grid=None):
+               rounds_state=None, groups=1, deferred=None, audit=None, keep_workspace=None, bound_grid=None,
+               bound_vertices=None):
     lib = _lib.lib()
     n = origins.shape[0]
     dev = origins.device
@@ -165,21 +174,25 @@
         ws_bytes = (ctypes.c_size_t * G)(*[b for _, b in work])
         st_ptrs = (ctypes.c_void_p * G)(*[st.cuda_stream for st in streams])
         cells, cells_n = (_ptr(bound_grid), bound_grid.shape[0]) if bound_grid is not None else (None, 0)
+        vert_g, cell_l = (None, None) if bound_vertices is None else (_ptr(bound_vertices[0]), _ptr(bound_vertices[1]))
+        if bound_vertices is not None and (bound_grid is None or bound_vertices[0].shape[0] != cells_n + 1 or
+                                           bound_vertices[1].shape[0] != cells_n):
+            raise ValueError('bound_vertices: the arrays of build_bound_grid(vertices=True), with their bound_grid')
 
         def run(sel, r0, r1):
             if len(sel) == G and G > 1:
                 b_, w_, wb_, s_, c_ = begin, ws_ptrs, ws_bytes, st_ptrs, counters
-                call('nefii_trace_rays_groups_grid', ctypes.byref(pm_sdf.struct), ctypes.byref(params), _ptr(origins), _ptr(dirs),
+                call('nefii_trace_rays_groups_grid_vertices', ctypes.byref(pm_sdf.struct), ctypes.byref(params), _ptr(origins), _ptr(dirs),
                      _ptr(om), G, b_, _ptr(lin_steps), _ptr(minsdf_steps), _ptr(pts), _ptr(hit), _ptr(dist), w_, wb_,
-                     _ptr(c_) if c_ is not None else None, r0, r1, cells, cells_n, stream=s_)
+                     _ptr(c_) if c_ is not None else None, r0, r1, cells, cells_n, vert_g, cell_l, stream=s_)
                 return
             for g in sel:
                 lo, hi = bounds[g]
                 ws, nbytes = work[g]
-                call('nefii_trace_rays_rounds_grid', ctypes.byref(pm_sdf.struct), ctypes.byref(params), _ptr(origins[lo:hi]),
+                call('nefii_trace_rays_rounds_grid_vertices', ctypes.byref(pm_sdf.struct), ctypes.byref(params), _ptr(origins[lo:hi]),
                      _ptr(dirs[lo:hi]), _ptr(om[lo:hi]), hi - lo, _ptr(lin_steps), _ptr(minsdf_steps), _ptr(pts[lo:hi]),
                      _ptr(hit[lo:hi]), _ptr(dist[lo:hi]), _ptr(ws), nbytes, _ptr(counters[g]) if counters is not None else None,
-                     r0, r1, cells, cells_n, stream=streams[g].cuda_stream)
+                     r0, r1, cells, cells_n, vert_g, cell_l, stream=streams[g].cuda_stream)
 
         def join():
             for st in streams:
```
